# endernewton/tf-faster-rcnn

Measured on AMD Instinct MI355X. Metric: images/sec (600×1000) ResNet-101 Faster R-CNN at 1/2/4/8 MI355X, higher is better.
Workload: dtype f32 (operands, accumulators, results; GEMMs with Cin, Cout % 128 == 0 form each f32 product from two-piece fp16 operands with an exact power-of-two scale per 128-k block on the fp16 matrix pipe -- 3 MFMAs / product, dropped terms <= 3 * 2^-22, measured error vs float64 below the f32-MFMA kernel's; o

## Files before the change

### include/frcnn_hip.h

```cpp
#ifndef FRCNN_HIP_H_
#define FRCNN_HIP_H_
#include <stddef.h>
#include <stdint.h>

#ifdef __cplusplus
extern "C" {
#endif

#define FRCNN_OK 0
#define FRCNN_E_ARG (-1)
#define FRCNN_E_WS (-2)
#define FRCNN_E_UNSUPPORTED (-3)
#define FRCNN_E_HIP(e) (-(1000 + (int)(e)))

#define FRCNN_NMS_RULE_CPU 0
#define FRCNN_NMS_RULE_GPU 1

#define FRCNN_ACT_NONE 0
#define FRCNN_ACT_RELU 1
#define FRCNN_ACT_RELU6 2

#define FRCNN_ABI_VERSION 6
int frcnn_abi_version(void);
const char* frcnn_build_info(void);
// ... 63 lines not shown
int frcnn_detect_post_batched(const float* cls_prob_d, const float* bbox_pred_d, const float* rois_d, const int* num_rois_d,
                              int B, int R, int C, double im_scale, int im_h, int im_w, double nms_thresh, int rule,
                              float score_thresh, int max_per_image, float* out_dets_d, int* out_count_d, int max_out,
                              long long out_stride, void* ws, size_t ws_bytes, void* stream);

int frcnn_im_detect_boxes(const float* rois_d, const float* bbox_pred_d, int R, int C, double im_scale,
                          int im_h, int im_w, float* boxes_d, void* stream);

int frcnn_bbox_transform_inv(const float* boxes_d, const float* deltas_d, int N, int k, float* out_d, void* stream);
int frcnn_clip_boxes(float* boxes_d, int N, int k, float im_h, float im_w, void* stream);
int frcnn_bbox_transform(const float* ex_rois_d, const float* gt_rois_d, int N, float* targets_d, void* stream);

int frcnn_bbox_overlaps(const double* boxes_d, int n, const double* query_d, int k, double* out_d, void* stream);

size_t frcnn_coco_match_workspace_bytes(int n_groups, long long n_det, long long n_gt, long long n_pairs);
int frcnn_coco_match(const double* det_xywh_d, const long long* det_off_d, const double* gt_xywh_d, const double* gt_area_d,
                     const unsigned char* gt_crowd_d, const long long* gt_off_d, int n_groups, const double* iou_thrs_d, int T,
                     const double* area_rng_d, int A, unsigned char* det_matched_d, unsigned char* det_ignored_d,
                     unsigned char* gt_ignored_d, double* iou_out_d, void* ws, size_t ws_bytes, void* stream);

int frcnn_conv2d_nhwc(const float* x_d, int N, int H, int W, int Cin, const float* w_d, const float* bias_d,
                      const float* residual_d, int RH, int RW, int res_stride, float* y_d, int OH, int OW,
                      int Cout, int KH, int KW, int stride, int pad_top, int pad_left, int act, int fold_w,
                      void* stream);
size_t frcnn_conv2d_workspace_bytes(int N, int OH, int OW, int Cout, int KH, int KW, int Cin, int fold_w);
int frcnn_conv2d_nhwc_ws(const float* x_d, int N, int H, int W, int Cin, const float* w_d, const float* bias_d,
                         const float* residual_d, int RH, int RW, int res_stride, float* y_d, int OH, int OW, int Cout, int KH,
                         int KW, int stride, int pad_top, int pad_left, int act, int fold_w, void* ws, size_t ws_bytes,
                         void* stream);

int frcnn_set_tuning(int key, int value);
unsigned int frcnn_crc32c(const void* data, size_t n, unsigned int crc);

long long frcnn_snappy_uncompress(const unsigned char* src, size_t n, unsigned char* dst, size_t cap);

int frcnn_prep_image_shape(int h, int w, int target_size, int max_size, double* im_scale, int* out_h, int* out_w);
int frcnn_prep_image(const void* src_d, int src_is_float, int h, int w, const double* pixel_means, double im_scale, float* out_d,
                     int OH, int OW, int out_c, void* stream);
int frcnn_prep_image_batched(const void* src_d, int src_is_float, int B, int h, int w, const double* pixel_means, double im_scale,
                             float* out_d, int OH, int OW, int out_c, void* stream);
int frcnn_prep_train_image(const void* src_d, int src_is_float, int h, int w, int flipped, const double* pixel_means, double im_scale,
                           float* out_d, int OH, int OW, int out_c, const unsigned short* boxes_d, const int* classes_d, int G,
                           float* gt_d, void* stream);

int frcnn_jpeg_info(const unsigned char* data, size_t n, int* out8);
size_t frcnn_jpeg_coef_bytes(int width, int height, int ncomp, int hs, int vs);
int frcnn_jpeg_entropy_decode(const unsigned char* data, size_t n, void* coef_h, size_t coef_bytes);
int frcnn_jpeg_pixels_host(const void* coef_h, int width, int height, int ncomp, int hs, int vs, unsigned char* bgr_h);
size_t frcnn_jpeg_workspace_bytes(int width, int height, int ncomp, int hs, int vs);
int frcnn_jpeg_pixels(const void* coef_d, int width, int height, int ncomp, int hs, int vs, unsigned char* bgr_d, void* ws,
                      size_t ws_bytes, void* stream);

int frcnn_gemm_batched_nt(const float* x_d, const float* w_d, float* y_d, int G, int M, int N, int K, void* stream);
size_t frcnn_gemm_x3_pack_bytes(int G, int N, int K);
int frcnn_gemm_x3_pack(const float* w_d, int G, int N, int K, void* planes_d, void* stream);
int frcnn_gemm_x3(const float* x_d, const void* planes_d, const float* bias_d, const float* res_d, float* y_d, int G, int M, int N,
                  int K, int act, int cfg, int terms, void* stream);
size_t frcnn_h2_planes_bytes(long long rows, int K);
int frcnn_h2_pack_w(const float* w_d, int G, int N, int K, void* planes_d, float* w_inv_d, void* stream);
int frcnn_h2_split(const float* x_d, long long M, int K, void* planes_d, float* inv_d, void* stream);
int frcnn_gemm_h2(const void* x_planes_d, const float* x_inv_d, const void* w_planes_d, const float* w_inv_d, const float* bias_d,
                  const float* res_d, const void* res_planes_d, const float* res_inv_d, float* y_d, void* y_planes_d, float* y_inv_d,
                  int G, int M, int N, int K, int act, int cfg, void* stream);
size_t frcnn_gemm_h2_mean_workspace_bytes(int G, int M, int N);
int frcnn_gemm_h2_mean(const void* x_planes_d, const float* x_inv_d, const void* w_planes_d, const float* w_inv_d, const float* bias_d,
                       const float* res_d, const void* res_planes_d, const float* res_inv_d, int G, int M, int N, int K, int act, int rows,
                       float* mean_out_d, void* ws, size_t ws_bytes, int cfg, void* stream);
int frcnn_winograd_filter_transform(const float* w_hwio, int Cin, int Cout, const float* scale, int m, float* u_out);
int frcnn_winograd_filter_transform_device(const float* w_packed_d, int Cout, int Cin, int m, int transpose_flip, float* u_d,
                                           void* stream);
int frcnn_winograd_input_transform(const float* x_d, int N, int H, int W, int C, int m, float* v_d, void* stream);
int frcnn_winograd_output_transform(const float* m_d, int N, int H, int W, int C, int m, const float* bias_d, int act, float* y_d,
                                    void* stream);
int frcnn_winograd7_filter_transform(const float* w_hwio, int Cin, int Cout, const float* scale, float* u_out);
int frcnn_winograd7_filter_transform_device(const float* w_packed_d, int Cout, int Cin, int transpose_flip, float* u_d, void* stream);
int frcnn_winograd7_input_transform(const float* x_d, int R, int C, float* v_d, void* stream);
int frcnn_winograd7_output_transform(const float* m_d, int R, int C, const float* bias_d, int act, float* y_d, void* stream);
int frcnn_winograd_input_transform_h2(const float* x_d, int N, int H, int W, int C, int m, void* v_planes_d, float* v_inv_d, void* stream);
int frcnn_winograd_output_transform_h2(const float* m_d, int N, int H, int W, int C, int m, const float* bias_d, int act, float* y_d,
                                       void* y_planes_d, float* y_inv_d, void* stream);
int frcnn_winograd7_input_transform_h2(const float* x_d, int R, int C, void* v_planes_d, float* v_inv_d, void* stream);
int frcnn_winograd7_output_transform_h2(const float* m_d, int R, int C, const float* bias_d, int act, float* y_d, void* y_planes_d,
                                        float* y_inv_d, void* stream);
int frcnn_pack_filter_hwio(const float* w_hwio, int KH, int KW, int Cin, int Cout, const float* scale, float* out);
int frcnn_maxpool_nhwc(const float* x_d, int N, int H, int W, int C, int k, int stride, int pad_top,
                       int pad_left, float* y_d, int OH, int OW, void* stream);
int frcnn_dwconv3x3_nhwc(const float* x_d, int N, int H, int W, int C, const float* w_d, const float* bias_d,
                         float* y_d, int OH, int OW, int stride, int pad_top, int pad_left, int act, void* stream);
int frcnn_dwconv3x3_nhwc_h2(const float* x_d, int N, int H, int W, int C, const float* w_d, const float* bias_d, float* y_d,
                            void* y_planes_d, float* y_inv_d, int OH, int OW, int stride, int pad_top, int pad_left, int act, void* stream);
int frcnn_spatial_mean(const float* x_d, int N, int HW, int C, float* y_d, void* stream);
int frcnn_softmax_rows(const float* x_d, int R, int C, int ld, float* y_d, void* stream);
int frcnn_rpn_softmax(const float* score_d, int HW, int A, int ld, float* prob_d, void* stream);
int frcnn_copy_cols(const float* src_d, int R, int ld_src, int col0, int cols, float* dst_d, int ld_dst, void* stream);

size_t frcnn_anchor_target_workspace_bytes(int H, int W, int A, int max_gt);
int frcnn_anchor_target_layer(const float* gt_boxes_d, int G, float im_h, float im_w, int H, int W, int A,
                              int feat_stride, const double* base_d, int rpn_batchsize, double fg_fraction,
                              double pos_overlap, double neg_overlap, long long seed, const double* opts, float* labels_d,
                              float* bbox_targets_d, float* inside_w_d, float* outside_w_d, void* ws,
                              size_t ws_bytes, void* stream);
int frcnn_anchor_target_layer_inject(const float* gt_boxes_d, int G, float im_h, float im_w, int H, int W, int A, int feat_stride,
                                     const double* base_d, int rpn_batchsize, double fg_fraction, double pos_overlap,
                                     double neg_overlap, const int* disable_d, int n_disable, const double* opts, float* labels_d,
                                     float* bbox_targets_d, float* inside_w_d, float* outside_w_d, void* ws, size_t ws_bytes,
                                     void* stream);
int frcnn_proposal_target_layer(const float* rpn_rois_d, const float* rpn_scores_d, int N, const float* gt_boxes_d,
                                int G, int num_classes, int batch_size, double fg_fraction, double fg_thresh,
                                double bg_thresh_hi, double bg_thresh_lo, const double* means4, const double* stds4,
                                long long seed, const double* opts, float* rois_d, float* roi_scores_d, float* labels_d,
                                float* bbox_targets_d, float* inside_w_d, float* outside_w_d, int* counts_d,
                                void* stream);
int frcnn_proposal_target_layer_dn(const float* rpn_rois_d, const float* rpn_scores_d, int max_rois, const int* num_rois_d,
                                   const float* gt_boxes_d, int G, int num_classes, int batch_size, double fg_fraction,
                                   double fg_thresh, double bg_thresh_hi, double bg_thresh_lo, const double* means4,
                                   const double* stds4, long long seed, const double* opts, float* rois_d, float* roi_scores_d,
                                   float* labels_d, float* bbox_targets_d, float* inside_w_d, float* outside_w_d, int* counts_d,
                                   void* stream);
int frcnn_proposal_target_layer_inject(const float* rpn_rois_d, const float* rpn_scores_d, int N, const float* gt_boxes_d, int G,
                                       int num_classes, int batch_size, const int* keep_inds_d, int n_fg, const double* means4,
                                       const double* stds4, const double* opts, float* rois_d, float* roi_scores_d, float* labels_d,
                                       float* bbox_targets_d, float* inside_w_d, float* outside_w_d, void* stream);
size_t frcnn_loss_workspace_bytes(long long elements);
int frcnn_softmax_ce_loss(const float* logits_d, const float* labels_d, int R, int C, int rpn_A, int rpn_H, int rpn_W,
                          float* loss_d, float* dlogits_d, void* ws, size_t ws_bytes, void* stream);
int frcnn_smooth_l1_loss(const float* pred_d, const float* targets_d, const float* inside_w_d, const float* outside_w_d,
                         long long n, float sigma, float mean_divisor, float* loss_d, float* dpred_d, void* ws,
                         size_t ws_bytes, void* stream);

int frcnn_transpose_pad(const float* in_d, int M, int C, float* out_d, int Mp, void* stream);
int frcnn_im2col_t(const float* x_d, int N, int H, int W, int Cin, int OH, int OW, int KH, int KW, int stride,
                   int pad_top, int pad_left, float* out_d, int Mp, void* stream);
int frcnn_flip_transpose_filter(const float* w_d, int Cout, int KH, int KW, int Cin, float* out_d, void* stream);
int frcnn_conv2d_dgrad_strided(const float* dy_d, int N, int OH, int OW, int Cout, const float* w_d, int KH, int KW,
                               int Cin, int stride, int pad_top, int pad_left, float* dx_d, int H, int W,
                               int accumulate, void* stream);
int frcnn_conv2d_wgrad_supported(int Cin, int Cout);
size_t frcnn_conv2d_wgrad_workspace_bytes(int N, int OH, int OW, int Cin, int Cout, int KH, int KW);
int frcnn_conv2d_wgrad(const float* dy_d, const float* x_d, int N, int H, int W, int Cin, int OH, int OW, int Cout, int KH, int KW,
                       int stride, int pad_top, int pad_left, float* dw_d, void* ws, size_t ws_bytes, void* stream);
void frcnn_conv2d_wgrad_set_plan(int tile, int min_workgroups);
size_t frcnn_conv2d_wgrad_h2_workspace_bytes(int N, int OH, int OW, int Cin, int Cout, int KH, int KW);
int frcnn_conv2d_wgrad_h2(const float* dy_d, const float* x_d, int N, int H, int W, int Cin, int OH, int OW, int Cout, int KH, int KW,
                          int stride, int pad_top, int pad_left, float* dw_d, void* ws, size_t ws_bytes, void* stream);
void frcnn_conv2d_wgrad_h2_set_plan(int tile, int min_workgroups);
int frcnn_relu_bwd(float* grad_d, const float* y_d, long long n, void* stream);
int frcnn_conv2d_nhwc_masked_ws(const float* x_d, int N, int H, int W, int Cin, const float* w_d, const float* bias_d,
                                const float* residual_d, int RH, int RW, int res_stride, float* y_d, int OH, int OW,
                                int Cout, int KH, int KW, int stride, int pad_top, int pad_left, int act, const float* mask_d,
                                void* ws, size_t ws_bytes, void* stream);
int frcnn_gemm_h2_masked(const void* x_planes_d, const float* x_inv_d, const void* w_planes_d, const float* w_inv_d, const float* bias_d,
                         const float* res_d, const float* mask_d, float* y_d, void* y_planes_d, float* y_inv_d, int G, int M, int N, int K,
                         int act, int cfg, void* stream);
int frcnn_winograd_output_transform_masked(const float* m_d, int N, int H, int W, int C, int m, const float* mask_d, float* y_d,
                                           void* y_planes_d, float* y_inv_d, void* stream);
int frcnn_winograd7_output_transform_masked(const float* m_d, int R, int C, const float* mask_d, float* y_d, void* y_planes_d,
                                            float* y_inv_d, void* stream);
int frcnn_relu6_bwd(float* grad_d, const float* y_d, long long n, void* stream);
int frcnn_maxpool_bwd(const float* x_d, int N, int H, int W, int C, int k, int stride, const float* y_d, const float* dy_d,
                      int OH, int OW, float* dx_d, void* stream);
int frcnn_dropout(const float* x_d, long long n, unsigned long long seed, float keep_prob, float* y_d, void* stream);
int frcnn_dwconv3x3_dgrad(const float* g_d, int N, int OH, int OW, int C, const float* w_d, float* dx_d, int H, int W, int stride,
                          int pad_top, int pad_left, int accumulate, void* stream);
size_t frcnn_dwconv3x3_wgrad_workspace_bytes(int N, int OH, int OW, int C);
int frcnn_dwconv3x3_wgrad(const float* g_d, const float* x_d, int N, int H, int W, int C, int OH, int OW, int stride, int pad_top,
                          int pad_left, const float* scale_d, float* dw_d, void* ws, size_t ws_bytes, void* stream);
// ... 41 lines not shown
```

### tf-faster-rcnn_amd/csrc/detect_kernels.hip

```cpp
#include "common.h"

extern "C" int frcnn_generate_anchors(int base_size, const double* ratios, int n_ratios, const double* scales,
                                      int n_scales, double* out_base) {
  if (!ratios || !scales || !out_base || n_ratios <= 0 || n_scales <= 0 || base_size <= 0) return FRCNN_E_ARG;
  const double w = (double)base_size, h = (double)base_size;
  const double cx = 0.5 * (w - 1), cy = 0.5 * (h - 1);
  for (int r = 0; r < n_ratios; ++r) {
    const double ws = nearbyint(sqrt(w * h / ratios[r]));
    const double hs = nearbyint(ws * ratios[r]);
    const double x1 = cx - 0.5 * (ws - 1), y1 = cy - 0.5 * (hs - 1);
    const double x2 = cx + 0.5 * (ws - 1), y2 = cy + 0.5 * (hs - 1);
    const double aw = x2 - x1 + 1, ah = y2 - y1 + 1;
    const double acx = x1 + 0.5 * (aw - 1), acy = y1 + 0.5 * (ah - 1);
    for (int s = 0; s < n_scales; ++s) {
      const double sw = aw * scales[s], sh = ah * scales[s];
      double* o = out_base + 4 * ((size_t)r * n_scales + s);
      o[0] = acx - 0.5 * (sw - 1);
      o[1] = acy - 0.5 * (sh - 1);
      o[2] = acx + 0.5 * (sw - 1);
      o[3] = acy + 0.5 * (sh - 1);
    }
  }
  return FRCNN_OK;
}

__device__ __forceinline__ float4 anchor_at(const double* __restrict__ base, int n, int A, int W, int stride) {
  const int a = n % A, pix = n / A;
  const double sx = (double)((pix % W) * stride), sy = (double)((pix / W) * stride);
  const double* b = base + 4 * a;
  return make_float4((float)(b[0] + sx), (float)(b[1] + sy), (float)(b[2] + sx), (float)(b[3] + sy));
}

__global__ void k_anchors(const double* __restrict__ base, int A, int W, int stride, int N, float4* __restrict__ out) {
  const int n = blockIdx.x * blockDim.x + threadIdx.x;
  if (n < N) out[n] = anchor_at(base, n, A, W, stride);
}

extern "C" int frcnn_generate_anchors_pre(int height, int width, int feat_stride, const double* base_d, int A,
                                          float* anchors_d, void* stream) {
  if (!base_d || !anchors_d || height <= 0 || width <= 0 || A <= 0) return FRCNN_E_ARG;
  const int N = height * width * A;
  hipLaunchKernelGGL(k_anchors, dim3(cdiv(N, 256)), dim3(256), 0, (hipStream_t)stream, base_d, A, width,
                     feat_stride, N, (float4*)anchors_d);
  LAUNCH_CHECK();
  return FRCNN_OK;
}

#define NMS_RULE_CPU FRCNN_NMS_RULE_CPU
#define NMS_RULE_GPU FRCNN_NMS_RULE_GPU
#define NMS_RULE_TF 2

__global__ void k_decode_clip_key(const float* __restrict__ prob, const float4* __restrict__ deltas,
                                  const double* __restrict__ base, int A, int W, int stride, int N, float hi_x,
                                  float hi_y, float4* __restrict__ boxes, u64* __restrict__ keys, size_t img) {
  const int n = blockIdx.x * blockDim.x + threadIdx.x;
  if (n >= N) return;
  const int b = blockIdx.y;
  prob += (size_t)b * 2 * N;
  deltas += (size_t)b * N;
  const int a = n % A, pix = n / A;
  const float score = prob[(size_t)pix * 2 * A + A + a];
  float4 bx = decode_box(anchor_at(base, n, A, W, stride), deltas[n]);
  bx.x = rmax(rmin(bx.x, hi_x), 0.0f);
  bx.y = rmax(rmin(bx.y, hi_y), 0.0f);
  bx.z = rmax(rmin(bx.z, hi_x), 0.0f);
  bx.w = rmax(rmin(bx.w, hi_y), 0.0f);
  img_ptr(boxes, img, b)[n] = bx;
  img_ptr(keys, img, b)[n] = make_key(score, (u32)n);
}

__global__ void k_dets_key(const float* __restrict__ dets, int k, float4* __restrict__ boxes, u64* __restrict__ keys) {
  const int n = blockIdx.x * blockDim.x + threadIdx.x;
  if (n >= k) return;
  const float* d = dets + 5 * (size_t)n;
  boxes[n] = make_float4(d[0], d[1], d[2], d[3]);
  keys[n] = make_key(d[4], (u32)n);
}

__global__ void k_boxes_scores_key(const float4* __restrict__ in_boxes, const float* __restrict__ in_scores, int k,
                                   float4* __restrict__ boxes, u64* __restrict__ keys) {
  const int n = blockIdx.x * blockDim.x + threadIdx.x;
  if (n >= k) return;
  boxes[n] = in_boxes[n];
// ... 652 lines not shown
  if (!rpn_cls_prob_d || !rpn_bbox_pred_d || !base_d || !rois_d || !scores_d || !ws) return FRCNN_E_ARG;
  if (H <= 0 || W <= 0 || A <= 0 || rpn_top_n <= 0) return FRCNN_E_ARG;
  const int N = H * W * A;
  if (N < rpn_top_n) return FRCNN_E_UNSUPPORTED;
  hipStream_t st = (hipStream_t)stream;
  SortWs s = carve(ws, N, rpn_top_n);
  if (s.bytes > ws_bytes) return FRCNN_E_WS;
  int rc = launch_decode(s, rpn_cls_prob_d, rpn_bbox_pred_d, 1, im_h, im_w, W, A, feat_stride, base_d, N, st);
  if (rc) return rc;
  rc = launch_topk_sort(s, N, rpn_top_n, 1, st);
  if (rc) return rc;
  hipLaunchKernelGGL(k_top_rois, dim3(cdiv(rpn_top_n, 256)), dim3(256), 0, st, s.sboxes, s.sscores, rpn_top_n, rois_d,
                     scores_d);
  LAUNCH_CHECK();
  return FRCNN_OK;
}

extern "C" int frcnn_proposal_top_layer_inds(const float* rpn_cls_prob_d, const float* rpn_bbox_pred_d, float im_h, float im_w,
                                             int H, int W, int A, int feat_stride, const double* base_d, const int* top_inds_d,
                                             int n_inds, float* rois_d, float* scores_d, void* stream) {
  if (!rpn_cls_prob_d || !rpn_bbox_pred_d || !base_d || !rois_d || !scores_d || !top_inds_d) return FRCNN_E_ARG;
  if (H <= 0 || W <= 0 || A <= 0 || n_inds <= 0) return FRCNN_E_ARG;
  hipLaunchKernelGGL(k_decode_gather, dim3(cdiv(n_inds, 256)), dim3(256), 0, (hipStream_t)stream, rpn_cls_prob_d,
                     (const float4*)rpn_bbox_pred_d, base_d, A, W, feat_stride, H * W * A, im_w - 1.0f, im_h - 1.0f, top_inds_d, n_inds,
                     rois_d, scores_d);
  LAUNCH_CHECK();
  return FRCNN_OK;
}

extern "C" int frcnn_non_max_suppression(const float* boxes_d, const float* scores_d, int k, int max_output_size,
                                         float iou_threshold, int* selected_d, int* num_d, void* ws, size_t ws_bytes,
                                         void* stream) {
  if (!num_d || k < 0 || max_output_size < 0) return FRCNN_E_ARG;
  hipStream_t st = (hipStream_t)stream;
  if (k == 0 || max_output_size == 0) {
    HIP_TRY(hipMemsetAsync(num_d, 0, sizeof(int), st));
    return FRCNN_OK;
  }
  if (!boxes_d || !scores_d || !selected_d || !ws) return FRCNN_E_ARG;
  if (k > NMS_MAX_BOXES) return FRCNN_E_UNSUPPORTED;
  SortWs s = carve(ws, k, k);
  if (s.bytes > ws_bytes) return FRCNN_E_WS;
  hipLaunchKernelGGL(k_boxes_scores_key, dim3(cdiv(k, 256)), dim3(256), 0, st, (const float4*)boxes_d, scores_d, k, s.boxes,
                     s.keys);
  LAUNCH_CHECK();
  int rc = launch_topk_sort(s, k, k, 1, st);
  if (rc) return rc;
  rc = launch_mask(s, k, 1, iou_threshold, NMS_RULE_TF, st);
  if (rc) return rc;
  ReduceOut o = {s.sboxes, s.sscores, s.sidx, nullptr, nullptr, selected_d, num_d, 0};
  return launch_reduce(s, k, 1, min(max_output_size, k), o, st);
}

extern "C" int frcnn_proposal_layer_tf_batched(const float* rpn_cls_prob_d, const float* rpn_bbox_pred_d, int B, float im_h,
                                               float im_w, int H, int W, int A, int feat_stride, const double* base_d,
                                               int post_nms_topn, float nms_thresh, float* rois_d, float* scores_d, int* num_d,
                                               void* ws, size_t ws_bytes, void* stream) {
  if (!rpn_cls_prob_d || !rpn_bbox_pred_d || !base_d || !rois_d || !scores_d || !num_d || !ws) return FRCNN_E_ARG;
  if (B <= 0 || H <= 0 || W <= 0 || A <= 0 || post_nms_topn <= 0) return FRCNN_E_ARG;
  const long long NN = (long long)H * W * A;
  if (NN > NMS_MAX_BOXES) return FRCNN_E_UNSUPPORTED;
  const int N = (int)NN;
  hipStream_t st = (hipStream_t)stream;
  SortWs s = carve(ws, N, N);
  if (s.bytes * (size_t)B > ws_bytes) return FRCNN_E_WS;
  int rc = launch_decode(s, rpn_cls_prob_d, rpn_bbox_pred_d, B, im_h, im_w, W, A, feat_stride, base_d, N, st);
  if (rc) return rc;
  rc = launch_topk_sort(s, N, N, B, st);
  if (rc) return rc;
  rc = launch_mask(s, N, B, nms_thresh, NMS_RULE_TF, st);
  if (rc) return rc;
  ReduceOut o = {s.sboxes, s.sscores, s.sidx, rois_d, scores_d, nullptr, num_d, 1};
  return launch_reduce(s, N, B, post_nms_topn, o, st);
}

extern "C" int frcnn_proposal_layer_tf(const float* rpn_cls_prob_d, const float* rpn_bbox_pred_d, float im_h, float im_w,
                                       int H, int W, int A, int feat_stride, const double* base_d, int post_nms_topn,
                                       float nms_thresh, float* rois_d, float* scores_d, int* num_d, void* ws,
                                       size_t ws_bytes, void* stream) {
  return frcnn_proposal_layer_tf_batched(rpn_cls_prob_d, rpn_bbox_pred_d, 1, im_h, im_w, H, W, A, feat_stride, base_d, post_nms_topn,
                                         nms_thresh, rois_d, scores_d, num_d, ws, ws_bytes, stream);
}

__device__ __forceinline__ float4 lerp4(const float4 a, const float4 b, float t) {
  return make_float4(a.x + (b.x - a.x) * t, a.y + (b.y - a.y) * t, a.z + (b.z - a.z) * t, a.w + (b.w - a.w) * t);
}
__device__ __forceinline__ float4 max4(const float4 a, const float4 b) {
  return make_float4(fmaxf(a.x, b.x), fmaxf(a.y, b.y), fmaxf(a.z, b.z), fmaxf(a.w, b.w));
}

__device__ __forceinline__ float4 crop_sample(const float4* __restrict__ feat, int H, int W, int C4, int c4, float y1,
                                              float x1, float hs, float ws, int gy, int gx) {
  const float in_y = y1 * (float)(H - 1) + (float)gy * hs;
  const float in_x = x1 * (float)(W - 1) + (float)gx * ws;
  if (in_y < 0 || in_y > (float)(H - 1) || in_x < 0 || in_x > (float)(W - 1)) return make_float4(0, 0, 0, 0);
  const int top = (int)floorf(in_y), bot = (int)ceilf(in_y);
  const int left = (int)floorf(in_x), right = (int)ceilf(in_x);
  const float ly = in_y - (float)top, lx = in_x - (float)left;
  const float4 tl = feat[((size_t)top * W + left) * C4 + c4], tr = feat[((size_t)top * W + right) * C4 + c4];
  const float4 bl = feat[((size_t)bot * W + left) * C4 + c4], br = feat[((size_t)bot * W + right) * C4 + c4];
  return lerp4(lerp4(tl, tr, lx), lerp4(bl, br, lx), ly);
}

template <bool MAX2>
__global__ __launch_bounds__(256) void k_crop_and_resize(const float4* __restrict__ feat_all, int NIMG, int H, int W, int C4,
                                                         int nslab, const float* __restrict__ rois, float stride, int pool,
                                                         const float4* __restrict__ bias, int act, float4* __restrict__ out) {
  const int slab = blockIdx.x % nslab, rp = blockIdx.x / nslab;
  const int r = rp / pool, py = rp % pool;
  const int SC4 = C4 / nslab, c40 = slab * SC4;
  const float height = ((float)H - 1.0f) * stride, width = ((float)W - 1.0f) * stride;
  const float* roi = rois + 5 * (size_t)r;
  const int img = (int)roi[0];
  float4* orow = out + ((size_t)r * pool + py) * pool * C4;
  if (img < 0 || img >= NIMG) {
    for (int t = threadIdx.x; t < pool * SC4; t += 256) orow[(size_t)(t / SC4) * C4 + c40 + t % SC4] = make_float4(0, 0, 0, 0);
    return;
  }
  const float4* feat = feat_all + (size_t)img * H * W * C4;
  const float x1 = roi[1] / width, y1 = roi[2] / height, x2 = roi[3] / width, y2 = roi[4] / height;
  const int P = MAX2 ? 2 * pool : pool;
  const float hs = (y2 - y1) * (float)(H - 1) / (float)(P - 1);
  const float ws = (x2 - x1) * (float)(W - 1) / (float)(P - 1);
  for (int t = threadIdx.x; t < pool * SC4; t += 256) {
    const int px = t / SC4, c4 = c40 + t % SC4;
    float4 v;
    if (MAX2) {
      v = crop_sample(feat, H, W, C4, c4, y1, x1, hs, ws, 2 * py, 2 * px);
      v = max4(v, crop_sample(feat, H, W, C4, c4, y1, x1, hs, ws, 2 * py, 2 * px + 1));
      v = max4(v, crop_sample(feat, H, W, C4, c4, y1, x1, hs, ws, 2 * py + 1, 2 * px));
      v = max4(v, crop_sample(feat, H, W, C4, c4, y1, x1, hs, ws, 2 * py + 1, 2 * px + 1));
    } else {
      v = crop_sample(feat, H, W, C4, c4, y1, x1, hs, ws, py, px);
    }
    if (bias) {
      const float4 bv = bias[c4];
      v.x += bv.x; v.y += bv.y; v.z += bv.z; v.w += bv.w;
    }
    if (act == FRCNN_ACT_RELU) v = act_relu(v);
    orow[(size_t)px * C4 + c4] = v;
  }
}

template <bool MAX2, int ITEMS>
__global__ __launch_bounds__(256) void k_crop_and_resize_roi(const float4* __restrict__ feat_all, int NIMG, int H, int W, int C4,
                                                             int nslab, const float* __restrict__ rois, float stride, int pool,
                                                             const float4* __restrict__ bias, int act, float4* __restrict__ out) {
  const int slab = blockIdx.x % nslab, r = blockIdx.x / nslab;
  const int SC4 = C4 / nslab, c40 = slab * SC4;
  const float height = ((float)H - 1.0f) * stride, width = ((float)W - 1.0f) * stride;
  const float* roi = rois + 5 * (size_t)r;
  const int img = (int)roi[0];
  float4* obase = out + (size_t)r * pool * pool * C4;
  const int total = pool * pool * SC4;
  if (img < 0 || img >= NIMG) {
    for (int t = threadIdx.x; t < total; t += 256) obase[(size_t)(t / SC4) * C4 + c40 + t % SC4] = make_float4(0, 0, 0, 0);
    return;
  }
  const float4* feat = feat_all + (size_t)img * H * W * C4;
  const float x1 = roi[1] / width, y1 = roi[2] / height, x2 = roi[3] / width, y2 = roi[4] / height;
  const int P = MAX2 ? 2 * pool : pool;
  const float hs = (y2 - y1) * (float)(H - 1) / (float)(P - 1);
  const float ws = (x2 - x1) * (float)(W - 1) / (float)(P - 1);
  for (int t0 = threadIdx.x; t0 < total; t0 += 256 * ITEMS) {
    float4 v[ITEMS];
#pragma unroll
    for (int k = 0; k < ITEMS; ++k) {
      const int t = t0 + k * 256;
      if (t >= total) { v[k] = make_float4(0, 0, 0, 0); continue; }
      const int pix = t / SC4, c4 = c40 + t % SC4;
      const int py = pix / pool, px = pix - py * pool;
      if (MAX2) {
        v[k] = crop_sample(feat, H, W, C4, c4, y1, x1, hs, ws, 2 * py, 2 * px);
        v[k] = max4(v[k], crop_sample(feat, H, W, C4, c4, y1, x1, hs, ws, 2 * py, 2 * px + 1));
        v[k] = max4(v[k], crop_sample(feat, H, W, C4, c4, y1, x1, hs, ws, 2 * py + 1, 2 * px));
        v[k] = max4(v[k], crop_sample(feat, H, W, C4, c4, y1, x1, hs, ws, 2 * py + 1, 2 * px + 1));
      } else {
        v[k] = crop_sample(feat, H, W, C4, c4, y1, x1, hs, ws, py, px);
      }
    }
#pragma unroll
    for (int k = 0; k < ITEMS; ++k) {
      const int t = t0 + k * 256;
      if (t >= total) continue;
      const int pix = t / SC4, c4 = c40 + t % SC4;
      float4 o = v[k];
      if (bias) {
        const float4 bv = bias[c4];
        o.x += bv.x; o.y += bv.y; o.z += bv.z; o.w += bv.w;
      }
      if (act == FRCNN_ACT_RELU) o = act_relu(o);
      obase[(size_t)pix * C4 + c4] = o;
    }
  }
}

static thread_local int g_crop_slabs = -1;
static thread_local int g_crop_form = 0;

static int launch_crop(const float* feat_d, int NIMG, int H, int W, int C, const float* rois_d, int R, float feat_stride, int pool,
                       int fuse_max2x2, const float* bias_d, int act, float* out_d, void* stream) {
  if (R == 0) return FRCNN_OK;
  if (!feat_d || !rois_d || !out_d || NIMG <= 0 || H < 2 || W < 2 || C <= 0 || R < 0 || pool < 2) return FRCNN_E_ARG;
  if (C % 4) return FRCNN_E_UNSUPPORTED;
  hipStream_t st = (hipStream_t)stream;
  const int C4 = C / 4;
  int nslab = (C4 % 8 == 0 && C4 / 8 >= 16) ? 8 : 1;
  if (g_crop_form == 0 && nslab == 8 && C4 / 8 < 32) nslab = 4;
  if (g_crop_slabs > 0 && C4 % g_crop_slabs == 0) nslab = g_crop_slabs;
  const long long blocks = (long long)R * pool * nslab;
  if (blocks >= (1ll << 31)) return FRCNN_E_UNSUPPORTED;
  if (g_crop_form == 0) {
    const unsigned grid = (unsigned)((long long)R * nslab);
    if (fuse_max2x2)
      hipLaunchKernelGGL((k_crop_and_resize_roi<true, 2>), dim3(grid), dim3(256), 0, st, (const float4*)feat_d, NIMG, H, W, C4, nslab, rois_d,
                         feat_stride, pool, (const float4*)bias_d, act, (float4*)out_d);
    else
      hipLaunchKernelGGL((k_crop_and_resize_roi<false, 4>), dim3(grid), dim3(256), 0, st, (const float4*)feat_d, NIMG, H, W, C4, nslab, rois_d,
                         feat_stride, pool, (const float4*)bias_d, act, (float4*)out_d);
    LAUNCH_CHECK();
    return FRCNN_OK;
  }
  if (fuse_max2x2)
    hipLaunchKernelGGL(k_crop_and_resize<true>, dim3((unsigned)blocks), dim3(256), 0, st, (const float4*)feat_d, NIMG, H, W, C4, nslab,
                       rois_d, feat_stride, pool, (const float4*)bias_d, act, (float4*)out_d);
  else
    hipLaunchKernelGGL(k_crop_and_resize<false>, dim3((unsigned)blocks), dim3(256), 0, st, (const float4*)feat_d, NIMG, H, W, C4, nslab,
                       rois_d, feat_stride, pool, (const float4*)bias_d, act, (float4*)out_d);
  LAUNCH_CHECK();
  return FRCNN_OK;
}

extern "C" int frcnn_detect_set_tuning(int key, int value) {
  if (key == 4) { g_crop_slabs = value; return FRCNN_OK; }
  if (key == 5) { g_crop_form = value; return FRCNN_OK; }
  return FRCNN_E_ARG;
}

extern "C" int frcnn_crop_and_resize(const float* feat_d, int H, int W, int C, const float* rois_d, int R,
                                     float feat_stride, int pool, int fuse_max2x2, float* out_d, void* stream) {
  return launch_crop(feat_d, 1, H, W, C, rois_d, R, feat_stride, pool, fuse_max2x2, nullptr, FRCNN_ACT_NONE, out_d, stream);
}

extern "C" int frcnn_crop_and_resize_batched(const float* feat_d, int N, int H, int W, int C, const float* rois_d, int R,
                                             float feat_stride, int pool, int fuse_max2x2, float* out_d, void* stream) {
  return launch_crop(feat_d, N, H, W, C, rois_d, R, feat_stride, pool, fuse_max2x2, nullptr, FRCNN_ACT_NONE, out_d, stream);
}

extern "C" int frcnn_crop_and_resize_bias_act(const float* feat_d, int N, int H, int W, int C, const float* rois_d, int R,
                                              float feat_stride, int pool, const float* bias_d, int act, float* out_d,
                                              void* stream) {
  if (act != FRCNN_ACT_NONE && act != FRCNN_ACT_RELU) return FRCNN_E_ARG;
  return launch_crop(feat_d, N, H, W, C, rois_d, R, feat_stride, pool, 0, bias_d, act, out_d, stream);
}

__global__ void k_bbox_transform_inv(const float4* __restrict__ boxes, const float4* __restrict__ deltas, int N, int k,
                                     float4* __restrict__ out) {
  const long long t = (long long)blockIdx.x * blockDim.x + threadIdx.x;
  if (t >= (long long)N * k) return;
  out[t] = decode_box(boxes[t / k], deltas[t]);
}
__global__ void k_clip_boxes(float4* __restrict__ boxes, long long n, float hi_x, float hi_y) {
  const long long t = (long long)blockIdx.x * blockDim.x + threadIdx.x;
  if (t >= n) return;
  float4 b = boxes[t];
  b.x = rmax(rmin(b.x, hi_x), 0.0f); b.y = rmax(rmin(b.y, hi_y), 0.0f);
  b.z = rmax(rmin(b.z, hi_x), 0.0f); b.w = rmax(rmin(b.w, hi_y), 0.0f);
  boxes[t] = b;
}
__global__ void k_bbox_transform(const float4* __restrict__ ex, const float4* __restrict__ gt, int N, float4* __restrict__ out) {
  const int t = blockIdx.x * blockDim.x + threadIdx.x;
  if (t >= N) return;
  const float4 e = ex[t], g = gt[t];
  const float ew = (e.z - e.x) + 1.0f, eh = (e.w - e.y) + 1.0f;
  const float ecx = e.x + 0.5f * ew, ecy = e.y + 0.5f * eh;
  const float gw = (g.z - g.x) + 1.0f, gh = (g.w - g.y) + 1.0f;
  const float gcx = g.x + 0.5f * gw, gcy = g.y + 0.5f * gh;
  out[t] = make_float4((gcx - ecx) / ew, (gcy - ecy) / eh, logf(gw / ew), logf(gh / eh));
}

extern "C" int frcnn_bbox_transform_inv(const float* boxes_d, const float* deltas_d, int N, int k, float* out_d, void* stream) {
  if (N < 0 || k <= 0) return FRCNN_E_ARG;
  if (N == 0) return FRCNN_OK;
  if (!boxes_d || !deltas_d || !out_d) return FRCNN_E_ARG;
  const long long tot = (long long)N * k;
  hipLaunchKernelGGL(k_bbox_transform_inv, dim3((unsigned)((tot + 255) / 256)), dim3(256), 0, (hipStream_t)stream,
                     (const float4*)boxes_d, (const float4*)deltas_d, N, k, (float4*)out_d);
  LAUNCH_CHECK();
  return FRCNN_OK;
}
extern "C" int frcnn_clip_boxes(float* boxes_d, int N, int k, float im_h, float im_w, void* stream) {
// ... 299 lines not shown
```

### tf-faster-rcnn_amd/csrc/gemm_h2.hip

```cpp
#include "h2_common.h"
#include <mutex>
#include <type_traits>

typedef float f32x16 __attribute__((ext_vector_type(16)));
typedef _Float16 h8 __attribute__((ext_vector_type(8)));

#define LDS_AS __attribute__((address_space(3)))

struct GemmH2Params {
  const unsigned short* x; const float* x_inv; const unsigned short* w; const float* w_inv;
  const float* bias; const float* res; const unsigned short* resp; const float* resp_inv; float* y; unsigned short* yp; float* y_inv;
  int M, N, K, batch, act, nsteps, mtiles, ntiles;
  long long Mtot;
  int wshare;
  const float* mask;
  float* mean_part; int mean_rows;
};

__device__ __forceinline__ void h2_glds16(unsigned voff, const void* sbase, unsigned lds_base) {
  unsigned keep;
  asm volatile(
      "s_mov_b32 %0, m0\n\t"
      "s_mov_b32 m0, %3\n\t"
      "s_nop 0\n\t"
// ... 1028 lines not shown
  return FRCNN_OK;
}

template <int MASK>
static int h2_dispatch(const GemmH2Params& p, int cfg, hipStream_t st) {
  switch (cfg) {
    case 9: return launch_h2<128, 128, 64, 64, 2, 2, H2_SCALES_ONCE + MASK>(p, st);
    case 12: return launch_h2<64, 128, 32, 64, 2, 2, MASK>(p, st);
    case 21: return launch_h2<256, 128, 64, 64, 3, 2, H2_SCALES_ONCE + H2_PINGPONG + MASK>(p, st);
    case 30: return launch_h2<128, 128, 64, 64, 2, 2, H2_SCALES_ONCE + H2_LIGHT_BOUNDARY + MASK>(p, st);
    case 31: return launch_h2<128, 128, 64, 64, 2, 2, H2_SCALES_ONCE + H2_LIGHT_BOUNDARY + H2_STORE16 + MASK>(p, st);
    case 32: return launch_h2<128, 128, 64, 64, 2, 2, H2_SCALES_ONCE + H2_STORE16 + MASK>(p, st);
    case 33: return launch_h2<64, 128, 32, 64, 2, 2, H2_LIGHT_BOUNDARY + H2_STORE16 + MASK>(p, st);
    case 34: return launch_h2<256, 128, 64, 64, 3, 2, H2_SCALES_ONCE + H2_PINGPONG + H2_STORE16 + MASK>(p, st);
    case 40: return launch_h2<128, 128, 64, 64, 2, 2, H2_SCALES_ONCE + H2_LIGHT_BOUNDARY + H2_STORE16 + H2_DEFERRED + MASK>(p, st);
    case 41: return launch_h2<64, 128, 32, 64, 2, 2, H2_LIGHT_BOUNDARY + H2_STORE16 + H2_DEFERRED + MASK>(p, st);
  }
#ifdef FRCNN_ABLATION
  constexpr int CFG31 = H2_SCALES_ONCE + H2_LIGHT_BOUNDARY + H2_STORE16;
  if constexpr (MASK == 0) switch (cfg) {
    case 50: return launch_h2<128, 128, 64, 64, 2, 2, CFG31 + H2_NO_MFMA>(p, st);
    case 51: return launch_h2<128, 128, 64, 64, 2, 2, CFG31 + H2_NO_FRAG>(p, st);
    case 52: return launch_h2<128, 128, 64, 64, 2, 2, CFG31 + H2_NO_LOAD>(p, st);
    case 53: return launch_h2<128, 128, 64, 64, 2, 2, CFG31 + H2_NO_MFMA + H2_NO_FRAG>(p, st);
    case 54: return launch_h2<128, 128, 64, 64, 2, 2, CFG31 + H2_NO_FRAG + H2_NO_LOAD>(p, st);
    case 55: return launch_h2<128, 128, 64, 64, 2, 2, CFG31 + H2_NO_MFMA + H2_NO_FRAG + H2_NO_LOAD>(p, st);
  }
#endif
  return FRCNN_E_ARG;
}

static int run_h2(GemmH2Params& p, int cfg, hipStream_t st);

static GemmH2Params h2_params(const void* x_planes_d, const float* x_inv_d, const void* w_planes_d, const float* w_inv_d, const float* bias_d,
                              const float* res_d, const void* res_planes_d, const float* res_inv_d, float* y_d, void* y_planes_d, float* y_inv_d,
                              int G, int M, int N, int K, int act) {
  GemmH2Params p;
  p.x = (const unsigned short*)x_planes_d; p.x_inv = x_inv_d; p.w = (const unsigned short*)w_planes_d; p.w_inv = w_inv_d;
  p.bias = bias_d; p.res = res_d; p.resp = (const unsigned short*)res_planes_d; p.resp_inv = res_inv_d; p.y = y_d; p.yp = (unsigned short*)y_planes_d; p.y_inv = y_inv_d;
  p.M = M; p.N = N; p.K = K; p.batch = G; p.act = act; p.Mtot = (long long)G * M;
  p.nsteps = p.mtiles = p.ntiles = 0;
  p.mean_part = nullptr; p.mean_rows = 0; p.wshare = 0; p.mask = nullptr;
  return p;
}

extern "C" int frcnn_gemm_h2(const void* x_planes_d, const float* x_inv_d, const void* w_planes_d, const float* w_inv_d, const float* bias_d,
                             const float* res_d, const void* res_planes_d, const float* res_inv_d, float* y_d, void* y_planes_d, float* y_inv_d,
                             int G, int M, int N, int K, int act, int cfg, void* stream) {
  if (!x_planes_d || !x_inv_d || !w_planes_d || !w_inv_d || (!y_d && !y_planes_d) || (y_planes_d && !y_inv_d) || G <= 0 || M <= 0 || N <= 0 ||
      K <= 0 || act < 0 || act > 2 || (res_d && res_planes_d) || (res_planes_d && !res_inv_d))
    return FRCNN_E_ARG;
  const long long Mtot = (long long)G * M;
  if (K % H2_KB || N % 128 || 4ll * Mtot * K >= (1ll << 32) || 4ll * N * K >= (1ll << 32) ||
      (long long)M * N >= (1ll << 29))
    return FRCNN_E_UNSUPPORTED;
  GemmH2Params p = h2_params(x_planes_d, x_inv_d, w_planes_d, w_inv_d, bias_d, res_d, res_planes_d, res_inv_d, y_d, y_planes_d, y_inv_d, G, M, N, K, act);
  return run_h2(p, cfg, (hipStream_t)stream);
}

extern "C" int frcnn_gemm_h2_masked(const void* x_planes_d, const float* x_inv_d, const void* w_planes_d, const float* w_inv_d, const float* bias_d,
                                    const float* res_d, const float* mask_d, float* y_d, void* y_planes_d, float* y_inv_d, int G, int M, int N, int K,
                                    int act, int cfg, void* stream) {
  if (!x_planes_d || !x_inv_d || !w_planes_d || !w_inv_d || !mask_d || (!y_d && !y_planes_d) || (y_planes_d && !y_inv_d) || G <= 0 || M <= 0 ||
      N <= 0 || K <= 0 || act < 0 || act > 2)
    return FRCNN_E_ARG;
  const long long Mtot = (long long)G * M;
  if (K % H2_KB || N % 128 || 4ll * Mtot * K >= (1ll << 32) || 4ll * N * K >= (1ll << 32) || (long long)M * N >= (1ll << 29)) return FRCNN_E_UNSUPPORTED;
  GemmH2Params p = h2_params(x_planes_d, x_inv_d, w_planes_d, w_inv_d, bias_d, res_d, nullptr, nullptr, y_d, y_planes_d, y_inv_d, G, M, N, K, act);
  p.mask = mask_d;
  return run_h2(p, cfg, (hipStream_t)stream);
}

static int run_h2(GemmH2Params& p, int cfg, hipStream_t st) {
  const int G = p.batch, M = p.M, N = p.N, K = p.K;
  if (cfg < 0) {
    const long long mt256 = (M + 255) / 256;
#ifndef FRCNN_H2_PP_MIN_K
#define FRCNN_H2_PP_MIN_K 1024
#endif
    const int pp_min_k = ((cfg == -4 || cfg == -5 || cfg == -6) && !p.mean_part) ? 512 : FRCNN_H2_PP_MIN_K;
    const int pp_cfg = (cfg == -3 || cfg == -4 || (cfg == -6 && K < FRCNN_H2_PP_MIN_K)) ? 34 : 21;
    const bool pp = K >= pp_min_k && mt256 * 256 * 100 <= (long long)M * 104 && mt256 * (N / 128) * G >= 256;
    const bool tiny = (long long)((M + 127) / 128) * (N / 128) * G < 150;
    const bool de = cfg != -2 && cfg != -7 && !p.mean_part && !p.mask && ((p.resp && p.yp && !p.y) || cfg == -8);
    cfg = pp ? pp_cfg : tiny ? (cfg == -2 ? 12 : (de && cfg == -8) ? 41 : 33) : (cfg == -2 ? 9 : de ? 40 : 31);
  }
  if (p.mean_part && (cfg == 40 || cfg == 41)) cfg = cfg == 40 ? 31 : 33;
  return p.mask ? h2_dispatch<H2_MASKED>(p, cfg, st) : h2_dispatch<0>(p, cfg, st);
}

__global__ __launch_bounds__(256) void k_h2_mean_finish(const float* __restrict__ part, int G, int M, int N4, int rows, float4* __restrict__ out) {
  const long long t = (long long)blockIdx.x * blockDim.x + threadIdx.x;
  const int per = M / rows;
  if (t >= (long long)G * per * N4) return;
  const int n4 = (int)(t % N4);
  const long long gr = t / N4;
  const int g = (int)(gr / per), r = (int)(gr % per);
  const int nblk = (M + 31) >> 5;
  const int row0 = r * rows, row1 = row0 + rows - 1;
  float4 s = make_float4(0.f, 0.f, 0.f, 0.f);
  for (int b = row0 >> 5; b <= (row1 >> 5); ++b) {
    const int which = ((b << 5) / rows == r) ? 0 : 1;
    const float4 v = *(const float4*)(part + (((size_t)g * nblk + b) * 2 + which) * (size_t)N4 * 4 + (size_t)n4 * 4);
    s.x += v.x; s.y += v.y; s.z += v.z; s.w += v.w;
  }
  const float inv = 1.0f / (float)rows;
  out[t] = make_float4(s.x * inv, s.y * inv, s.z * inv, s.w * inv);
}

extern "C" size_t frcnn_gemm_h2_mean_workspace_bytes(int G, int M, int N) {
  if (G <= 0 || M <= 0 || N <= 0) return 256;
  return (size_t)G * (size_t)((M + 31) / 32) * 2 * (size_t)N * sizeof(float);
}

extern "C" int frcnn_gemm_h2_mean(const void* x_planes_d, const float* x_inv_d, const void* w_planes_d, const float* w_inv_d, const float* bias_d,
                                  const float* res_d, const void* res_planes_d, const float* res_inv_d, int G, int M, int N, int K, int act, int rows,
                                  float* mean_out_d, void* ws, size_t ws_bytes, int cfg, void* stream) {
  if (!x_planes_d || !x_inv_d || !w_planes_d || !w_inv_d || !mean_out_d || !ws || G <= 0 || M <= 0 || N <= 0 || K <= 0 || act < 0 || act > 2 ||
      rows <= 0 || (res_d && res_planes_d) || (res_planes_d && !res_inv_d))
    return FRCNN_E_ARG;
  const long long Mtot = (long long)G * M;
  if (K % H2_KB || N % 128 || M % rows || rows < 32 || 4ll * Mtot * K >= (1ll << 32) || 4ll * N * K >= (1ll << 32) || (long long)M * N >= (1ll << 29))
    return FRCNN_E_UNSUPPORTED;
  if (frcnn_gemm_h2_mean_workspace_bytes(G, M, N) > ws_bytes) return FRCNN_E_WS;
  GemmH2Params p = h2_params(x_planes_d, x_inv_d, w_planes_d, w_inv_d, bias_d, res_d, res_planes_d, res_inv_d, nullptr, nullptr, nullptr, G, M, N, K, act);
  p.mean_part = (float*)ws; p.mean_rows = rows; p.wshare = 1;
  hipStream_t st = (hipStream_t)stream;
  const int rc = run_h2(p, cfg, st);
  if (rc) return rc;
  const long long tot = (long long)G * (M / rows) * (N / 4);
  hipLaunchKernelGGL(k_h2_mean_finish, dim3((unsigned)((tot + 255) / 256)), dim3(256), 0, st, (const float*)ws, G, M, N / 4, rows, (float4*)mean_out_d);
  LAUNCH_CHECK();
  return FRCNN_OK;
}
```

### tf-faster-rcnn_amd/csrc/winograd7.hip

```cpp
#include "h2_common.h"

namespace w7 {
constexpr float BT[11][9] = {
    {4.f, 0.f, -5.f, 0.f, 1.f, 0.f, 0.f, 0.f, 0.f},  {0.f, -4.f, -4.f, 1.f, 1.f, 0.f, 0.f, 0.f, 0.f}, {0.f, 4.f, -4.f, -1.f, 1.f, 0.f, 0.f, 0.f, 0.f},
    {0.f, -2.f, -1.f, 2.f, 1.f, 0.f, 0.f, 0.f, 0.f}, {0.f, 2.f, -1.f, -2.f, 1.f, 0.f, 0.f, 0.f, 0.f}, {0.f, 4.f, 0.f, -5.f, 0.f, 1.f, 0.f, 0.f, 0.f},
    {0.f, 0.f, 0.f, 0.f, 2.f, -1.f, -2.f, 1.f, 0.f}, {0.f, 0.f, 0.f, 0.f, 0.f, -2.f, -1.f, 1.f, 0.f}, {0.f, 0.f, 0.f, 0.f, 0.f, 2.f, -3.f, 1.f, 0.f},
    {0.f, 0.f, 0.f, 0.f, 0.f, -1.f, 0.f, 1.f, 0.f},  {0.f, 0.f, 0.f, 0.f, 0.f, 2.f, -1.f, -2.f, 1.f}};
constexpr float AT[7][11] = {
    {1.f, 1.f, 1.f, 1.f, 1.f, 0.f, 0.f, 0.f, 0.f, 0.f, 0.f},  {0.f, 1.f, -1.f, 2.f, -2.f, 0.f, 0.f, 0.f, 0.f, 0.f, 0.f},
    {0.f, 1.f, 1.f, 4.f, 4.f, 0.f, 0.f, 0.f, 0.f, 0.f, 0.f},  {0.f, 1.f, -1.f, 8.f, -8.f, 1.f, 0.f, 0.f, 0.f, 0.f, 0.f},
    {0.f, 0.f, 0.f, 0.f, 0.f, 0.f, 1.f, 1.f, 1.f, 1.f, 0.f},  {0.f, 0.f, 0.f, 0.f, 0.f, 0.f, 0.f, 1.f, -1.f, 2.f, 0.f},
    {0.f, 0.f, 0.f, 0.f, 0.f, 0.f, 0.f, 1.f, 1.f, 4.f, 1.f}};
constexpr double G[11][3] = {{1.0 / 4, 0, 0},          {-1.0 / 6, -1.0 / 6, -1.0 / 6}, {-1.0 / 6, 1.0 / 6, -1.0 / 6}, {1.0 / 24, 1.0 / 12, 1.0 / 6},
                             {1.0 / 24, -1.0 / 12, 1.0 / 6}, {0, 0, 1},                {1.0 / 2, 0, 0},               {-1.0 / 2, -1.0 / 2, -1.0 / 2},
                             {-1.0 / 6, 1.0 / 6, -1.0 / 6},  {1.0 / 6, 1.0 / 3, 2.0 / 3}, {0, 0, 1}};
}

__device__ __forceinline__ float2 f2mad(float a, float2 x, float2 y) { return make_float2(a * x.x + y.x, a * x.y + y.y); }

__device__ __forceinline__ void acc_term(float2& acc, bool& first, float coef, const float2 x) {
  if (coef == 0.f) return;
  if (first) {
    acc = coef == 1.f ? x : (coef == -1.f ? make_float2(-x.x, -x.y) : make_float2(coef * x.x, coef * x.y));
    first = false;
  } else if (coef == 1.f) {
    acc = make_float2(acc.x + x.x, acc.y + x.y);
  } else if (coef == -1.f) {
    acc = make_float2(acc.x - x.x, acc.y - x.y);
  } else {
    acc = f2mad(coef, x, acc);
  }
}

template <bool H2>
struct Wino7Sink {
  float2* f; unsigned short* planes; float* inv; size_t rows;
  template <int NR>
  __device__ __forceinline__ void putn(const size_t* row, const float2* v, int c2, int C2) const {
    if (!H2 || f) {
#pragma unroll
      for (int n = 0; n < NR; ++n) f[row[n] * C2 + c2] = v[n];
    }
    if (H2) {
      size_t e[NR];
      float* slot[NR];
#pragma unroll
      for (int n = 0; n < NR; ++n) {
        e[n] = (row[n] * C2 + c2) * 2;
        slot[n] = inv + (size_t)(c2 >> 6) * rows + row[n];
      }
      h2_emit_rows64<NR>(v, e, slot, (1u << NR) - 1u, planes, rows * (size_t)C2 * 2, c2 & 63);
    }
  }
};

template <bool H2>
__global__ void __launch_bounds__(256) k_wino7_input(const float2* __restrict__ x, int R, int C2, const Wino7Sink<H2> V) {
  const long long id = (long long)blockIdx.x * blockDim.x + threadIdx.x;
  if (id >= (long long)R * C2) return;
  const int c2 = (int)(id % C2);
  const int r = (int)(id / C2);
  float2 d[7][7];
  const float2* src = x + (size_t)r * 49 * C2 + c2;
#pragma unroll
  for (int i = 0; i < 7; ++i)
#pragma unroll
    for (int j = 0; j < 7; ++j) d[i][j] = src[(size_t)(i * 7 + j) * C2];
#pragma unroll
  for (int xi = 0; xi < 11; ++xi) {
    float2 t[7];
#pragma unroll
    for (int j = 0; j < 7; ++j) {
      bool first = true;
      t[j] = make_float2(0.f, 0.f);
#pragma unroll
      for (int i = 0; i < 7; ++i) acc_term(t[j], first, w7::BT[xi][i + 1], d[i][j]);
    }
    float2 o[11];
    size_t rw[11];
#pragma unroll
    for (int nu = 0; nu < 11; ++nu) {
      bool first = true;
      float2 v = make_float2(0.f, 0.f);
#pragma unroll
      for (int j = 0; j < 7; ++j) acc_term(v, first, w7::BT[nu][j + 1], t[j]);
      o[nu] = v;
      rw[nu] = (size_t)(xi * 11 + nu) * R + r;
    }
    V.template putn<11>(rw, o, c2, C2);
  }
}

template <int XI0, int NXI, int I0, int NI, bool H2, bool MASK>
__device__ __forceinline__ void wino7_out_segment(const float2* __restrict__ in, size_t plane, float2 bv, int act, const Wino7Sink<H2>& y,
                                                  size_t row0, int c2, int C2, const float2* __restrict__ mask) {
  float2 m[NXI][11];
#pragma unroll
  for (int a = 0; a < NXI; ++a)
#pragma unroll
    for (int nu = 0; nu < 11; ++nu) m[a][nu] = in[(size_t)((XI0 + a) * 11 + nu) * plane];
#pragma unroll
  for (int i = 0; i < NI; ++i) {
    float2 s[11];
#pragma unroll
    for (int nu = 0; nu < 11; ++nu) {
      bool first = true;
      s[nu] = make_float2(0.f, 0.f);
#pragma unroll
      for (int a = 0; a < NXI; ++a) acc_term(s[nu], first, w7::AT[I0 + i][XI0 + a], m[a][nu]);
    }
    float2 o[7];
    size_t rw[7];
#pragma unroll
    for (int j = 0; j < 7; ++j) {
      bool first = true;
      float2 v = make_float2(0.f, 0.f);
#pragma unroll
      for (int nu = 0; nu < 11; ++nu) acc_term(v, first, w7::AT[j][nu], s[nu]);
      v = make_float2(v.x + bv.x, v.y + bv.y);
      if (act == FRCNN_ACT_RELU) v = act_relu(v);
      rw[j] = row0 + (I0 + i) * 7 + j;
      if (MASK) {
        const float2 k = mask[rw[j] * C2 + c2];
        v.x = k.x > 0.f ? v.x : 0.f; v.y = k.y > 0.f ? v.y : 0.f;
      }
      o[j] = v;
    }
    y.template putn<7>(rw, o, c2, C2);
  }
}

template <bool H2, bool MASK = false>
__global__ void __launch_bounds__(256) k_wino7_output(const float2* __restrict__ Mx, int R, int C2, const float2* __restrict__ bias, int act,
                                                       const float2* __restrict__ mask, const Wino7Sink<H2> y) {
  const long long id = (long long)blockIdx.x * blockDim.x + threadIdx.x;
  if (id >= (long long)R * C2) return;
  const int c2 = (int)(id % C2);
  const int r = (int)(id / C2);
  const size_t plane = (size_t)R * C2;
  const float2* in = Mx + (size_t)r * C2 + c2;
  const float2 bv = bias ? bias[c2] : make_float2(0.f, 0.f);
  wino7_out_segment<0, 6, 0, 4, H2, MASK>(in, plane, bv, act, y, (size_t)r * 49, c2, C2, mask);
  wino7_out_segment<6, 5, 4, 3, H2, MASK>(in, plane, bv, act, y, (size_t)r * 49, c2, C2, mask);
}

__global__ void k_wino7_filter(const float* __restrict__ w, int O, int C, int transpose_flip, float* __restrict__ U) {
  const long long id = (long long)blockIdx.x * blockDim.x + threadIdx.x;
  if (id >= (long long)O * C) return;
  int o, c;
  if (transpose_flip) { o = (int)(id % O); c = (int)(id / O); }
  else { c = (int)(id % C); o = (int)(id / C); }
  float g[3][3];
#pragma unroll
  for (int i = 0; i < 3; ++i)
#pragma unroll
    for (int j = 0; j < 3; ++j) {
      const int kh = transpose_flip ? 2 - i : i, kw = transpose_flip ? 2 - j : j;
      g[i][j] = w[(((size_t)o * 3 + kh) * 3 + kw) * C + c];
    }
  float t[11][3];
#pragma unroll
  for (int a = 0; a < 11; ++a)
#pragma unroll
    for (int j = 0; j < 3; ++j) t[a][j] = (float)w7::G[a][0] * g[0][j] + (float)w7::G[a][1] * g[1][j] + (float)w7::G[a][2] * g[2][j];
  const size_t plane = (size_t)O * C;
  float* out = U + (transpose_flip ? (size_t)c * O + o : (size_t)o * C + c);
#pragma unroll
  for (int a = 0; a < 11; ++a)
#pragma unroll
    for (int b = 0; b < 11; ++b)
      out[(size_t)(a * 11 + b) * plane] = t[a][0] * (float)w7::G[b][0] + t[a][1] * (float)w7::G[b][1] + t[a][2] * (float)w7::G[b][2];
}

extern "C" int frcnn_winograd7_filter_transform(const float* w_hwio, int Cin, int Cout, const float* scale, float* u_out) {
  if (!w_hwio || !u_out || Cin <= 0 || Cout <= 0) return FRCNN_E_ARG;
  for (int c = 0; c < Cin; ++c)
    for (int o = 0; o < Cout; ++o) {
      double g[3][3], t[11][3];
      const double sc = scale ? (double)scale[o] : 1.0;
      for (int i = 0; i < 3; ++i)
        for (int j = 0; j < 3; ++j) g[i][j] = (double)w_hwio[((size_t)(i * 3 + j) * Cin + c) * Cout + o] * sc;
      for (int a = 0; a < 11; ++a)
        for (int j = 0; j < 3; ++j) t[a][j] = w7::G[a][0] * g[0][j] + w7::G[a][1] * g[1][j] + w7::G[a][2] * g[2][j];
      for (int a = 0; a < 11; ++a)
        for (int b = 0; b < 11; ++b)
          u_out[((size_t)(a * 11 + b) * Cout + o) * Cin + c] = (float)(t[a][0] * w7::G[b][0] + t[a][1] * w7::G[b][1] + t[a][2] * w7::G[b][2]);
    }
  return FRCNN_OK;
}

extern "C" int frcnn_winograd7_filter_transform_device(const float* w_packed_d, int Cout, int Cin, int transpose_flip, float* u_d,
                                                       void* stream) {
  if (!w_packed_d || !u_d || Cout <= 0 || Cin <= 0) return FRCNN_E_ARG;
  const long long tot = (long long)Cout * Cin;
  hipLaunchKernelGGL(k_wino7_filter, dim3((unsigned)((tot + 255) / 256)), dim3(256), 0, (hipStream_t)stream, w_packed_d, Cout, Cin,
                     transpose_flip ? 1 : 0, u_d);
  LAUNCH_CHECK();
  return FRCNN_OK;
}

extern "C" int frcnn_winograd7_input_transform(const float* x_d, int R, int C, float* v_d, void* stream) {
  if (!x_d || !v_d || R <= 0 || C <= 0) return FRCNN_E_ARG;
  if (C % 2) return FRCNN_E_UNSUPPORTED;
  const long long tot = (long long)R * (C / 2);
  const Wino7Sink<false> sink{(float2*)v_d, nullptr, nullptr, 0};
  hipLaunchKernelGGL(k_wino7_input<false>, dim3((unsigned)((tot + 255) / 256)), dim3(256), 0, (hipStream_t)stream, (const float2*)x_d, R, C / 2, sink);
  LAUNCH_CHECK();
  return FRCNN_OK;
}

extern "C" int frcnn_winograd7_input_transform_h2(const float* x_d, int R, int C, void* v_planes_d, float* v_inv_d, void* stream) {
  if (!x_d || !v_planes_d || !v_inv_d || R <= 0 || C <= 0) return FRCNN_E_ARG;
  if (C % H2_KB) return FRCNN_E_UNSUPPORTED;
  const long long tot = (long long)R * (C / 2);
  const Wino7Sink<true> sink{nullptr, (unsigned short*)v_planes_d, v_inv_d, (size_t)121 * R};
  hipLaunchKernelGGL(k_wino7_input<true>, dim3((unsigned)((tot + 255) / 256)), dim3(256), 0, (hipStream_t)stream, (const float2*)x_d, R, C / 2, sink);
  LAUNCH_CHECK();
  return FRCNN_OK;
}

extern "C" int frcnn_winograd7_output_transform(const float* m_d, int R, int C, const float* bias_d, int act, float* y_d, void* stream) {
  if (!m_d || !y_d || R <= 0 || C <= 0) return FRCNN_E_ARG;
  if (C % 2 || (act != FRCNN_ACT_NONE && act != FRCNN_ACT_RELU)) return FRCNN_E_UNSUPPORTED;
  const long long tot = (long long)R * (C / 2);
  const Wino7Sink<false> sink{(float2*)y_d, nullptr, nullptr, 0};
  hipLaunchKernelGGL((k_wino7_output<false, false>), dim3((unsigned)((tot + 255) / 256)), dim3(256), 0, (hipStream_t)stream, (const float2*)m_d, R,
                     C / 2, (const float2*)bias_d, act, (const float2*)nullptr, sink);
  LAUNCH_CHECK();
  return FRCNN_OK;
}

extern "C" int frcnn_winograd7_output_transform_h2(const float* m_d, int R, int C, const float* bias_d, int act, float* y_d, void* y_planes_d,
                                                   float* y_inv_d, void* stream) {
  if (!m_d || !y_planes_d || !y_inv_d || R <= 0 || C <= 0) return FRCNN_E_ARG;
  if (C % H2_KB || (act != FRCNN_ACT_NONE && act != FRCNN_ACT_RELU)) return FRCNN_E_UNSUPPORTED;
  const long long tot = (long long)R * (C / 2);
  const Wino7Sink<true> sink{(float2*)y_d, (unsigned short*)y_planes_d, y_inv_d, (size_t)R * 49};
  hipLaunchKernelGGL((k_wino7_output<true, false>), dim3((unsigned)((tot + 255) / 256)), dim3(256), 0, (hipStream_t)stream, (const float2*)m_d, R,
                     C / 2, (const float2*)bias_d, act, (const float2*)nullptr, sink);
  LAUNCH_CHECK();
  return FRCNN_OK;
}

extern "C" int frcnn_winograd7_output_transform_masked(const float* m_d, int R, int C, const float* mask_d, float* y_d, void* y_planes_d,
                                                       float* y_inv_d, void* stream) {
  if (!m_d || !mask_d || (!y_d && !y_planes_d) || (y_planes_d && !y_inv_d) || R <= 0 || C <= 0) return FRCNN_E_ARG;
  if (C % 2 || (y_planes_d && C % H2_KB)) return FRCNN_E_UNSUPPORTED;
  const long long tot = (long long)R * (C / 2);
  if (y_planes_d) {
    const Wino7Sink<true> sink{(float2*)y_d, (unsigned short*)y_planes_d, y_inv_d, (size_t)R * 49};
    hipLaunchKernelGGL((k_wino7_output<true, true>), dim3((unsigned)((tot + 255) / 256)), dim3(256), 0, (hipStream_t)stream, (const float2*)m_d, R,
                       C / 2, (const float2*)nullptr, FRCNN_ACT_NONE, (const float2*)mask_d, sink);
  } else {
    const Wino7Sink<false> sink{(float2*)y_d, nullptr, nullptr, 0};
    hipLaunchKernelGGL((k_wino7_output<false, true>), dim3((unsigned)((tot + 255) / 256)), dim3(256), 0, (hipStream_t)stream, (const float2*)m_d, R,
                       C / 2, (const float2*)nullptr, FRCNN_ACT_NONE, (const float2*)mask_d, sink);
  }
  LAUNCH_CHECK();
  return FRCNN_OK;
}
```

### tf-faster-rcnn_amd/frcnn_hip/__init__.py

```python
import ctypes
import os
from ctypes import c_double, c_float, c_int, c_longlong, c_size_t, c_ulonglong, c_void_p

_PKG = os.path.dirname(os.path.abspath(__file__))
LIB_PATH = os.path.join(_PKG, "libfrcnn_hip.so")
_lib = None

ABI_VERSION = 6
ACT_NONE, ACT_RELU, ACT_RELU6 = 0, 1, 2
NMS_RULE_CPU, NMS_RULE_GPU = 0, 1

_P = c_void_p
SIGNATURES = {
    "frcnn_abi_version": (c_int, []),
    "frcnn_build_info": (ctypes.c_char_p, []),
    "_nms": (None, [_P, _P, _P, c_int, c_int, c_float, c_int]),
    "frcnn_nms_workspace_bytes": (c_size_t, [c_int]),
    "frcnn_nms": (c_int, [_P, c_int, c_double, c_int, _P, _P, _P, c_size_t, _P]),
    "frcnn_nms_sorted": (c_int, [_P, c_int, c_int, c_double, c_int, _P, _P, _P, c_size_t, _P]),
    "frcnn_nms_rule": (c_int, [_P, c_int, c_double, c_int, c_int, _P, _P, _P, c_size_t, _P]),
    "frcnn_nms_sorted_rule": (c_int, [_P, c_int, c_int, c_double, c_int, c_int, _P, _P, _P, c_size_t, _P]),
    "frcnn_generate_anchors": (c_int, [c_int, _P, c_int, _P, c_int, _P]),
    "frcnn_generate_anchors_pre": (c_int, [c_int, c_int, c_int, _P, c_int, _P, _P]),
    "frcnn_proposal_workspace_bytes": (c_size_t, [c_int, c_int, c_int, c_int]),
    "frcnn_proposal_layer": (c_int, [_P, _P, c_float, c_float, c_int, c_int, c_int, c_int, _P, c_int, c_int, c_double,
                                     _P, _P, _P, _P, c_size_t, _P]),
    "frcnn_proposal_batched_workspace_bytes": (c_size_t, [c_int, c_int, c_int, c_int, c_int]),
    "frcnn_proposal_layer_batched": (c_int, [_P, _P, c_int, c_float, c_float, c_int, c_int, c_int, c_int, _P, c_int, c_int, c_double,
                                             c_int, _P, _P, _P, _P, c_size_t, _P]),
    "frcnn_proposal_top_layer_inds": (c_int, [_P, _P, c_float, c_float, c_int, c_int, c_int, c_int, _P, _P, c_int, _P, _P, _P]),
    "frcnn_proposal_layer_tf_batched": (c_int, [_P, _P, c_int, c_float, c_float, c_int, c_int, c_int, c_int, _P, c_int, c_float, _P, _P,
                                                _P, _P, c_size_t, _P]),
    "frcnn_proposal_top_layer": (c_int, [_P, _P, c_float, c_float, c_int, c_int, c_int, c_int, _P, c_int, _P, _P, _P,
                                         c_size_t, _P]),
    "frcnn_non_max_suppression": (c_int, [_P, _P, c_int, c_int, c_float, _P, _P, _P, c_size_t, _P]),
    "frcnn_proposal_layer_tf": (c_int, [_P, _P, c_float, c_float, c_int, c_int, c_int, c_int, _P, c_int, c_float, _P, _P, _P,
                                        _P, c_size_t, _P]),
    "frcnn_crop_and_resize": (c_int, [_P, c_int, c_int, c_int, _P, c_int, c_float, c_int, c_int, _P, _P]),
    "frcnn_crop_and_resize_batched": (c_int, [_P, c_int, c_int, c_int, c_int, _P, c_int, c_float, c_int, c_int, _P, _P]),
    "frcnn_crop_and_resize_bias_act": (c_int, [_P, c_int, c_int, c_int, c_int, _P, c_int, c_float, c_int, _P, c_int, _P, _P]),
    "frcnn_detect_set_tuning": (c_int, [c_int, c_int]),
    "frcnn_detect_post_batched_workspace_bytes": (c_size_t, [c_int, c_int, c_int]),
    "frcnn_detect_post_batched": (c_int, [_P, _P, _P, _P, c_int, c_int, c_int, c_double, c_int, c_int, c_double, c_int, c_float, c_int,
                                          _P, _P, c_int, c_longlong, _P, c_size_t, _P]),
    "frcnn_detect_post_workspace_bytes": (c_size_t, [c_int, c_int]),
    "frcnn_detect_post": (c_int, [_P, _P, _P, _P, c_int, c_int, c_double, c_int, c_int, c_double, c_float, c_int, _P, _P,
                                  c_int, _P, c_size_t, _P]),
    "frcnn_im_detect_boxes": (c_int, [_P, _P, c_int, c_int, c_double, c_int, c_int, _P, _P]),
    "frcnn_bbox_overlaps": (c_int, [_P, c_int, _P, c_int, _P, _P]),
    "frcnn_coco_match_workspace_bytes": (c_size_t, [c_int, c_longlong, c_longlong, c_longlong]),
    "frcnn_coco_match": (c_int, [_P, _P, _P, _P, _P, _P, c_int, _P, c_int, _P, c_int, _P, _P, _P, _P, _P, c_size_t, _P]),
    "frcnn_bbox_transform_inv": (c_int, [_P, _P, c_int, c_int, _P, _P]),
    "frcnn_clip_boxes": (c_int, [_P, c_int, c_int, c_float, c_float, _P]),
    "frcnn_bbox_transform": (c_int, [_P, _P, c_int, _P, _P]),
    "frcnn_conv2d_nhwc": (c_int, [_P, c_int, c_int, c_int, c_int, _P, _P, _P, c_int, c_int, c_int, _P, c_int, c_int,
                                  c_int, c_int, c_int, c_int, c_int, c_int, c_int, c_int, _P]),
    "frcnn_conv2d_workspace_bytes": (c_size_t, [c_int, c_int, c_int, c_int, c_int, c_int, c_int, c_int]),
    "frcnn_conv2d_nhwc_ws": (c_int, [_P, c_int, c_int, c_int, c_int, _P, _P, _P, c_int, c_int, c_int, _P, c_int, c_int,
                                     c_int, c_int, c_int, c_int, c_int, c_int, c_int, c_int, _P, c_size_t, _P]),
    "frcnn_conv2d_nhwc_masked_ws": (c_int, [_P, c_int, c_int, c_int, c_int, _P, _P, _P, c_int, c_int, c_int, _P, c_int, c_int,
                                            c_int, c_int, c_int, c_int, c_int, c_int, c_int, _P, _P, c_size_t, _P]),
    "frcnn_gemm_h2_masked": (c_int, [_P, _P, _P, _P, _P, _P, _P, _P, _P, _P, c_int, c_int, c_int, c_int, c_int, c_int, _P]),
    "frcnn_winograd_output_transform_masked": (c_int, [_P, c_int, c_int, c_int, c_int, c_int, _P, _P, _P, _P, _P]),
    "frcnn_winograd7_output_transform_masked": (c_int, [_P, c_int, c_int, _P, _P, _P, _P, _P]),
    "frcnn_crc32c": (ctypes.c_uint32, [_P, c_size_t, ctypes.c_uint32]),
    "frcnn_snappy_uncompress": (c_longlong, [_P, c_size_t, _P, c_size_t]),
    "frcnn_prep_image_shape": (c_int, [c_int, c_int, c_int, c_int, _P, _P, _P]),
    "frcnn_prep_image": (c_int, [_P, c_int, c_int, c_int, _P, c_double, _P, c_int, c_int, c_int, _P]),
    "frcnn_prep_image_batched": (c_int, [_P, c_int, c_int, c_int, c_int, _P, c_double, _P, c_int, c_int, c_int, _P]),
    "frcnn_prep_train_image": (c_int, [_P, c_int, c_int, c_int, c_int, _P, c_double, _P, c_int, c_int, c_int, _P, _P, c_int, _P, _P]),
    "frcnn_jpeg_info": (c_int, [_P, c_size_t, _P]),
    "frcnn_jpeg_coef_bytes": (c_size_t, [c_int, c_int, c_int, c_int, c_int]),
    "frcnn_jpeg_entropy_decode": (c_int, [_P, c_size_t, _P, c_size_t]),
    "frcnn_jpeg_pixels_host": (c_int, [_P, c_int, c_int, c_int, c_int, c_int, _P]),
    "frcnn_jpeg_workspace_bytes": (c_size_t, [c_int, c_int, c_int, c_int, c_int]),
    "frcnn_jpeg_pixels": (c_int, [_P, c_int, c_int, c_int, c_int, c_int, _P, _P, c_size_t, _P]),
    "frcnn_gemm_batched_nt": (c_int, [_P, _P, _P, c_int, c_int, c_int, c_int, _P]),
    "frcnn_winograd_filter_transform": (c_int, [_P, c_int, c_int, _P, c_int, _P]),
    "frcnn_winograd_filter_transform_device": (c_int, [_P, c_int, c_int, c_int, c_int, _P, _P]),
    "frcnn_winograd_input_transform": (c_int, [_P, c_int, c_int, c_int, c_int, c_int, _P, _P]),
    "frcnn_winograd_output_transform": (c_int, [_P, c_int, c_int, c_int, c_int, c_int, _P, c_int, _P, _P]),
    "frcnn_winograd7_filter_transform": (c_int, [_P, c_int, c_int, _P, _P]),
    "frcnn_winograd7_filter_transform_device": (c_int, [_P, c_int, c_int, c_int, _P, _P]),
    "frcnn_winograd7_input_transform": (c_int, [_P, c_int, c_int, _P, _P]),
    "frcnn_winograd7_output_transform": (c_int, [_P, c_int, c_int, _P, c_int, _P, _P]),
    "frcnn_winograd_input_transform_h2": (c_int, [_P, c_int, c_int, c_int, c_int, c_int, _P, _P, _P]),
    "frcnn_winograd_output_transform_h2": (c_int, [_P, c_int, c_int, c_int, c_int, c_int, _P, c_int, _P, _P, _P, _P]),
    "frcnn_winograd7_input_transform_h2": (c_int, [_P, c_int, c_int, _P, _P, _P]),
    "frcnn_winograd7_output_transform_h2": (c_int, [_P, c_int, c_int, _P, c_int, _P, _P, _P, _P]),
    "frcnn_set_tuning": (c_int, [c_int, c_int]),
    "frcnn_pack_filter_hwio": (c_int, [_P, c_int, c_int, c_int, c_int, _P, _P]),
    "frcnn_maxpool_nhwc": (c_int, [_P, c_int, c_int, c_int, c_int, c_int, c_int, c_int, c_int, _P, c_int, c_int, _P]),
    "frcnn_dwconv3x3_nhwc": (c_int, [_P, c_int, c_int, c_int, c_int, _P, _P, _P, c_int, c_int, c_int, c_int, c_int, c_int, _P]),
    "frcnn_dwconv3x3_nhwc_h2": (c_int, [_P, c_int, c_int, c_int, c_int, _P, _P, _P, _P, _P, c_int, c_int, c_int, c_int, c_int, c_int, _P]),
    "frcnn_spatial_mean": (c_int, [_P, c_int, c_int, c_int, _P, _P]),
    "frcnn_softmax_rows": (c_int, [_P, c_int, c_int, c_int, _P, _P]),
    "frcnn_rpn_softmax": (c_int, [_P, c_int, c_int, c_int, _P, _P]),
    "frcnn_copy_cols": (c_int, [_P, c_int, c_int, c_int, c_int, _P, c_int, _P]),
    "frcnn_anchor_target_workspace_bytes": (c_size_t, [c_int, c_int, c_int, c_int]),
    "frcnn_anchor_target_layer": (c_int, [_P, c_int, c_float, c_float, c_int, c_int, c_int, c_int, _P, c_int, c_double, c_double,
                                          c_double, c_longlong, _P, _P, _P, _P, _P, _P, c_size_t, _P]),
    "frcnn_anchor_target_layer_inject": (c_int, [_P, c_int, c_float, c_float, c_int, c_int, c_int, c_int, _P, c_int, c_double, c_double,
                                                 c_double, _P, c_int, _P, _P, _P, _P, _P, _P, c_size_t, _P]),
    "frcnn_proposal_target_layer_inject": (c_int, [_P, _P, c_int, _P, c_int, c_int, c_int, _P, c_int, _P, _P, _P, _P, _P, _P, _P, _P, _P, _P]),
    "frcnn_proposal_target_layer": (c_int, [_P, _P, c_int, _P, c_int, c_int, c_int, c_double, c_double, c_double, c_double, _P, _P,
                                            c_longlong, _P, _P, _P, _P, _P, _P, _P, _P, _P]),
    "frcnn_proposal_target_layer_dn": (c_int, [_P, _P, c_int, _P, _P, c_int, c_int, c_int, c_double, c_double, c_double, c_double, _P, _P,
                                               c_longlong, _P, _P, _P, _P, _P, _P, _P, _P, _P]),
    "frcnn_loss_workspace_bytes": (c_size_t, [c_longlong]),
    "frcnn_softmax_ce_loss": (c_int, [_P, _P, c_int, c_int, c_int, c_int, c_int, _P, _P, _P, c_size_t, _P]),
    "frcnn_smooth_l1_loss": (c_int, [_P, _P, _P, _P, c_longlong, c_float, c_float, _P, _P, _P, c_size_t, _P]),
    "frcnn_transpose_pad": (c_int, [_P, c_int, c_int, _P, c_int, _P]),
    "frcnn_im2col_t": (c_int, [_P, c_int, c_int, c_int, c_int, c_int, c_int, c_int, c_int, c_int, c_int, c_int, _P, c_int, _P]),
    "frcnn_flip_transpose_filter": (c_int, [_P, c_int, c_int, c_int, c_int, _P, _P]),
    "frcnn_conv2d_dgrad_strided": (c_int, [_P, c_int, c_int, c_int, c_int, _P, c_int, c_int, c_int, c_int, c_int, c_int, _P, c_int,
                                           c_int, c_int, _P]),
    "frcnn_conv2d_wgrad_supported": (c_int, [c_int, c_int]),
    "frcnn_conv2d_wgrad_workspace_bytes": (c_size_t, [c_int, c_int, c_int, c_int, c_int, c_int, c_int]),
    "frcnn_conv2d_wgrad": (c_int, [_P, _P, c_int, c_int, c_int, c_int, c_int, c_int, c_int, c_int, c_int, c_int, c_int, c_int, _P, _P,
                                   c_size_t, _P]),
    "frcnn_conv2d_wgrad_set_plan": (None, [c_int, c_int]),
    "frcnn_conv2d_wgrad_h2_workspace_bytes": (c_size_t, [c_int, c_int, c_int, c_int, c_int, c_int, c_int]),
    "frcnn_conv2d_wgrad_h2": (c_int, [_P, _P, c_int, c_int, c_int, c_int, c_int, c_int, c_int, c_int, c_int, c_int, c_int, c_int, _P, _P,
                                      c_size_t, _P]),
    "frcnn_conv2d_wgrad_h2_set_plan": (None, [c_int, c_int]),
    "frcnn_relu_bwd": (c_int, [_P, _P, c_longlong, _P]),
    "frcnn_gemm_x3_pack_bytes": (c_size_t, [c_int, c_int, c_int]),
    "frcnn_gemm_x3_pack": (c_int, [_P, c_int, c_int, c_int, _P, _P]),
    "frcnn_gemm_x3": (c_int, [_P, _P, _P, _P, _P, c_int, c_int, c_int, c_int, c_int, c_int, c_int, _P]),
    "frcnn_h2_planes_bytes": (c_size_t, [c_longlong, c_int]),
    "frcnn_h2_pack_w": (c_int, [_P, c_int, c_int, c_int, _P, _P, _P]),
    "frcnn_h2_split": (c_int, [_P, c_longlong, c_int, _P, _P, _P]),
    "frcnn_gemm_h2": (c_int, [_P, _P, _P, _P, _P, _P, _P, _P, _P, _P, _P, c_int, c_int, c_int, c_int, c_int, c_int, _P]),
    "frcnn_gemm_h2_mean_workspace_bytes": (c_size_t, [c_int, c_int, c_int]),
    "frcnn_gemm_h2_mean": (c_int, [_P, _P, _P, _P, _P, _P, _P, _P, c_int, c_int, c_int, c_int, c_int, c_int, _P, _P, c_size_t, c_int, _P]),
    "frcnn_relu6_bwd": (c_int, [_P, _P, c_longlong, _P]),
    "frcnn_maxpool_bwd": (c_int, [_P, c_int, c_int, c_int, c_int, c_int, c_int, _P, _P, c_int, c_int, _P, _P]),
    "frcnn_dropout": (c_int, [_P, c_longlong, c_ulonglong, c_float, _P, _P]),
    "frcnn_dwconv3x3_dgrad": (c_int, [_P, c_int, c_int, c_int, c_int, _P, _P, c_int, c_int, c_int, c_int, c_int, c_int, _P]),
    "frcnn_dwconv3x3_wgrad_workspace_bytes": (c_size_t, [c_int, c_int, c_int, c_int]),
    "frcnn_dwconv3x3_wgrad": (c_int, [_P, _P, c_int, c_int, c_int, c_int, c_int, c_int, c_int, c_int, c_int, _P, _P, _P, c_size_t, _P]),
    "frcnn_dwconv3x3_refold": (c_int, [_P, _P, c_int, _P, _P]),
    "frcnn_add_strided": (c_int, [_P, c_int, c_int, c_int, c_int, _P, c_int, c_int, c_int, c_int, _P]),
    "frcnn_spatial_mean_bwd": (c_int, [_P, c_int, c_int, c_int, _P, _P]),
    "frcnn_colsum": (c_int, [_P, c_int, c_int, _P, _P]),
    "frcnn_crop_and_resize_bwd": (c_int, [_P, c_int, c_int, c_int, _P, c_int, c_float, c_int, _P, _P]),
    "frcnn_crop_and_resize_bwd_plan": (c_int, [_P, c_int, c_int, c_int, _P, c_int, c_float, c_int, _P, c_size_t, _P]),
    "frcnn_sgd_momentum": (c_int, [_P, _P, _P, _P, _P, c_longlong, c_int, c_float, c_float, c_float, c_float, _P]),
    "frcnn_sgd_desc_bytes": (c_size_t, []),
    "frcnn_sgd_momentum_multi": (c_int, [_P, c_int, c_float, c_float, c_float, _P]),
    "frcnn_sgd_momentum_range": (c_int, [_P, c_int, c_int, c_float, c_float, c_float, _P]),
    "frcnn_sumsq": (c_int, [_P, c_longlong, c_double, _P, c_int, _P, c_size_t, _P]),
    "frcnn_sumsq_multi": (c_int, [_P, _P, c_int, c_double, _P, c_int, _P, c_size_t, _P]),
    "frcnn_summary_limits": (c_int, [_P]),
    "frcnn_summary_stats_workspace_bytes": (c_size_t, [c_int]),
    "frcnn_summary_stats": (c_int, [_P, c_int, _P, _P, c_size_t, _P]),
    "frcnn_graph_begin": (c_int, [_P]),
    "frcnn_graph_end": (c_int, [_P, ctypes.POINTER(c_void_p)]),
    "frcnn_graph_launch": (c_int, [_P, _P]),
    "frcnn_graph_destroy": (c_int, [_P]),
}


class FrcnnHipError(RuntimeError):
    pass


def lib():
    global _lib
    if _lib is None:
        if not os.path.exists(LIB_PATH):
            raise ImportError("libfrcnn_hip.so not built: run `python -c 'import __graft_entry__ as g; g.build()'` "
# ... 30 lines not shown
```

### tf-faster-rcnn_amd/frcnn_hip/ops.py

```python
import ctypes

import numpy as np
import torch

import frcnn_hip as _binding
from . import ACT_NONE, NMS_RULE_CPU, call, lib

_ws_cache = {}
ws_scope = "default"

_scope_stack = [(None, None, None)]


def active_store(owner, default=None):
    o, _, store = _scope_stack[-1]
    return store if store is not None and (owner is None or o is owner) else default


def scope_depth():
    return len(_scope_stack) - 1


class unscoped(object):

# ... 231 lines not shown
    return out


def proposal_layer(rpn_cls_prob, rpn_bbox_pred, im_h, im_w, feat_stride, base_d, pre_nms_topn, post_nms_topn,
                   nms_thresh, rois=None, scores=None, num=None, rule=NMS_RULE_CPU):
    _chk(rpn_cls_prob), _chk(rpn_bbox_pred), _chk(base_d, torch.float64)
    B, H, W, A2 = rpn_cls_prob.shape
    A = A2 // 2
    dev = rpn_cls_prob.device
    rois = _empty((B * post_nms_topn, 5), dtype=torch.float32, device=dev) if rois is None else rois
    scores = _empty((B * post_nms_topn, 1), dtype=torch.float32, device=dev) if scores is None else scores
    num = _zeros((B,), dtype=torch.int32, device=dev) if num is None else num
    nb = lib().frcnn_proposal_batched_workspace_bytes(B, H, W, A, int(pre_nms_topn))
    ws = workspace(nb, dev, "proposal")
    call("frcnn_proposal_layer_batched", _ptr(rpn_cls_prob), _ptr(rpn_bbox_pred), B, float(im_h), float(im_w), H, W, A,
         int(feat_stride), _ptr(base_d), int(pre_nms_topn), int(post_nms_topn), float(nms_thresh), int(rule), _ptr(rois),
         _ptr(scores), _ptr(num), _ptr(ws), ws.numel(), _stream())
    return rois, scores, num


def proposal_layer_tf(rpn_cls_prob, rpn_bbox_pred, im_h, im_w, feat_stride, base_d, post_nms_topn, nms_thresh, rois=None,
                      scores=None, num=None):
    _chk(rpn_cls_prob), _chk(rpn_bbox_pred), _chk(base_d, torch.float64)
    B, H, W, A2 = rpn_cls_prob.shape
    A = A2 // 2
    dev = rpn_cls_prob.device
    rois = _empty((B * post_nms_topn, 5), dtype=torch.float32, device=dev) if rois is None else rois
    scores = _empty((B * post_nms_topn, 1), dtype=torch.float32, device=dev) if scores is None else scores
    num = _zeros((B,), dtype=torch.int32, device=dev) if num is None else num
    nb = lib().frcnn_proposal_batched_workspace_bytes(B, H, W, A, 0)
    ws = workspace(nb, dev, "proposal")
    call("frcnn_proposal_layer_tf_batched", _ptr(rpn_cls_prob), _ptr(rpn_bbox_pred), B, float(im_h), float(im_w), H, W, A,
         int(feat_stride), _ptr(base_d), int(post_nms_topn), float(nms_thresh), _ptr(rois), _ptr(scores), _ptr(num),
         _ptr(ws), ws.numel(), _stream())
    return rois, scores, num


def proposal_top_layer_inds(rpn_cls_prob, rpn_bbox_pred, im_h, im_w, feat_stride, base_d, top_inds, rois=None, scores=None):
    _chk(rpn_cls_prob), _chk(rpn_bbox_pred), _chk(base_d, torch.float64), _chk(top_inds, torch.int32)
    _, H, W, A2 = rpn_cls_prob.shape
    n = top_inds.numel()
    dev = rpn_cls_prob.device
    rois = _empty((n, 5), dtype=torch.float32, device=dev) if rois is None else rois
    scores = _empty((n, 1), dtype=torch.float32, device=dev) if scores is None else scores
    call("frcnn_proposal_top_layer_inds", _ptr(rpn_cls_prob), _ptr(rpn_bbox_pred), float(im_h), float(im_w), H, W, A2 // 2,
         int(feat_stride), _ptr(base_d), _ptr(top_inds), n, _ptr(rois), _ptr(scores), _stream())
    return rois, scores


def proposal_top_layer(rpn_cls_prob, rpn_bbox_pred, im_h, im_w, feat_stride, base_d, rpn_top_n, rois=None, scores=None):
    _chk(rpn_cls_prob), _chk(rpn_bbox_pred), _chk(base_d, torch.float64)
    _, H, W, A2 = rpn_cls_prob.shape
    A = A2 // 2
    dev = rpn_cls_prob.device
    rois = _empty((rpn_top_n, 5), dtype=torch.float32, device=dev) if rois is None else rois
    scores = _empty((rpn_top_n, 1), dtype=torch.float32, device=dev) if scores is None else scores
    nb = lib().frcnn_proposal_workspace_bytes(H, W, A, int(rpn_top_n))
    ws = workspace(nb, dev, "proposal")
    call("frcnn_proposal_top_layer", _ptr(rpn_cls_prob), _ptr(rpn_bbox_pred), float(im_h), float(im_w), H, W, A,
         int(feat_stride), _ptr(base_d), int(rpn_top_n), _ptr(rois), _ptr(scores), _ptr(ws), ws.numel(), _stream())
    return rois, scores


def crop_and_resize(feat, rois, feat_stride, pool, max_pool=False, out=None):
    _chk(feat), _chk(rois)
    H, W, C = feat.shape[-3:]
    N = feat.shape[0] if feat.dim() == 4 else 1
    R = rois.shape[0]
    out = _empty((R, pool, pool, C), dtype=torch.float32, device=feat.device) if out is None else out
    call("frcnn_crop_and_resize_batched", _ptr(feat), N, H, W, C, _ptr(rois), R, float(feat_stride), int(pool),
         1 if max_pool else 0, _ptr(out), _stream())
    return out


def crop_and_resize_bias_act(feat, rois, feat_stride, pool, bias, act, out=None):
    _chk(feat), _chk(rois)
    H, W, C = feat.shape[-3:]
    N = feat.shape[0] if feat.dim() == 4 else 1
    R = rois.shape[0]
    out = _empty((R, pool, pool, C), dtype=torch.float32, device=feat.device) if out is None else out
    call("frcnn_crop_and_resize_bias_act", _ptr(feat), N, H, W, C, _ptr(rois), R, float(feat_stride), int(pool), _ptr(bias),
         int(act), _ptr(out), _stream())
    return out


def detect_post(cls_prob, bbox_pred, rois, num_rois, im_scale, im_h, im_w, nms_thresh=0.3, score_thresh=0.0,
                max_per_image=100, max_out=None, out=None, count=None, batch=1, rule=NMS_RULE_CPU):
    _chk(cls_prob), _chk(rois)
    if bbox_pred is not None:
        _chk(bbox_pred)
    B = int(batch)
    R, C = cls_prob.shape[0] // B, cls_prob.shape[1]
    if cls_prob.shape[0] != B * R or rois.shape[0] != B * R:
        raise ValueError("detect_post: %d rows do not split into %d images" % (cls_prob.shape[0], B))
    dev = cls_prob.device
    max_out = (max_per_image + 28 if max_per_image > 0 else R * (C - 1)) if max_out is None else max_out
    shape = (max_out, 6) if B == 1 else (B, max_out, 6)
    out = _empty(shape, dtype=torch.float32, device=dev) if out is None else out
    count = _zeros((B,), dtype=torch.int32, device=dev) if count is None else count
    if out.dtype != torch.float32 or out.shape[-1] != 6 or out.stride(-1) != 1 or out.stride(-2) != 6 or out.shape[-2] < max_out:
        raise ValueError("detect_post: `out` must be float32 [.., >=max_out, 6] with contiguous images")
    out_stride = out.stride(0) if out.dim() == 3 else 0
    nb = lib().frcnn_detect_post_batched_workspace_bytes(B, R, C)
    ws = workspace(nb, dev, "detect_post")
    call("frcnn_detect_post_batched", _ptr(cls_prob), _ptr(bbox_pred), _ptr(rois), _ptr(num_rois), B, R, C, float(im_scale),
         int(im_h), int(im_w), float(nms_thresh), int(rule), float(score_thresh), int(max_per_image), _ptr(out), _ptr(count),
         int(max_out), int(out_stride), _ptr(ws), ws.numel(), _stream())
    return out, count


def im_detect_boxes(rois, bbox_pred, im_scale, im_h, im_w, num_classes=None):
    _chk(rois)
    if bbox_pred is None:
        R, C4 = rois.shape[0], 4 * int(num_classes)
    else:
        _chk(bbox_pred)
        R, C4 = bbox_pred.shape
    out = _empty((R, C4), dtype=torch.float32, device=rois.device)
    call("frcnn_im_detect_boxes", _ptr(rois), _ptr(bbox_pred), R, C4 // 4, float(im_scale), int(im_h), int(im_w), _ptr(out),
         _stream())
    return out


def pack_filter_hwio(w_hwio, scale=None):
    w = np.ascontiguousarray(w_hwio, dtype=np.float32)
    KH, KW, Cin, Cout = w.shape
    out = np.empty((Cout, KH, KW, Cin), dtype=np.float32)
    sc = None if scale is None else np.ascontiguousarray(scale, dtype=np.float32)
    call("frcnn_pack_filter_hwio", w.ctypes.data_as(ctypes.c_void_p), KH, KW, Cin, Cout,
         None if sc is None else sc.ctypes.data_as(ctypes.c_void_p), out.ctypes.data_as(ctypes.c_void_p))
    return out


def pack_filter_foldw(w_hwio, scale=None):
    w = np.asarray(w_hwio, dtype=np.float32)
    KH, KW, Cin, Cout = w.shape
    assert KW <= 8 and Cin <= 4
    if scale is not None:
        w = w * np.asarray(scale, dtype=np.float32)[None, None, None, :]
    out = np.zeros((Cout, KH, 8, 4), dtype=np.float32)
    out[:, :, :KW, :Cin] = np.transpose(w, (3, 0, 1, 2))
    return out


def conv_out_size(n, k, stride, pad_lo, pad_hi):
    return (n + pad_lo + pad_hi - k) // stride + 1


split_k = True


def conv2d(x, w_packed, bias, KH, KW, stride=1, pad=(0, 0, 0, 0), act=ACT_NONE, residual=None, res_stride=1,
           fold_w=False, out=None, mask=None):
    _chk(x), _chk(w_packed)
    N, H, W, Cin = x.shape
    Cout = w_packed.shape[0]
    OH = conv_out_size(H, KH, stride, pad[0], pad[1])
    OW = conv_out_size(W, KW, stride, pad[2], pad[3])
    out = _empty((N, OH, OW, Cout), dtype=torch.float32, device=x.device) if out is None else out
    RH = RW = 0
    if residual is not None:
        _chk(residual)
        RH, RW = residual.shape[1], residual.shape[2]
    nb = lib().frcnn_conv2d_workspace_bytes(N, OH, OW, Cout, KH, KW, Cin, 1 if fold_w else 0) if split_k else 0
    if mask is not None:
        _chk(mask)
# ... 138 lines not shown
    sc = None if scale is None else np.ascontiguousarray(scale, dtype=np.float32)
    if m == 7:
        out = np.empty((121, Cout, Cin), dtype=np.float32)
        call("frcnn_winograd7_filter_transform", w.ctypes.data_as(ctypes.c_void_p), Cin, Cout,
             None if sc is None else sc.ctypes.data_as(ctypes.c_void_p), out.ctypes.data_as(ctypes.c_void_p))
        return out
    out = np.empty(((m + 2) ** 2, Cout, Cin), dtype=np.float32)
    call("frcnn_winograd_filter_transform", w.ctypes.data_as(ctypes.c_void_p), Cin, Cout,
         None if sc is None else sc.ctypes.data_as(ctypes.c_void_p), int(m), out.ctypes.data_as(ctypes.c_void_p))
    return out


def winograd_filter_transform_device(w_packed, m=4, transpose_flip=False, out=None):
    _chk(w_packed)
    O, kh, kw, C = w_packed.shape
    assert kh == 3 and kw == 3
    G = winograd_points(m)
    shape = (G, C, O) if transpose_flip else (G, O, C)
    out = _empty(shape, dtype=torch.float32, device=w_packed.device) if out is None else out
    assert out.numel() == G * O * C
    if m == 7:
        call("frcnn_winograd7_filter_transform_device", _ptr(w_packed), O, C, 1 if transpose_flip else 0, _ptr(out), _stream())
    else:
        call("frcnn_winograd_filter_transform_device", _ptr(w_packed), O, C, int(m), 1 if transpose_flip else 0, _ptr(out), _stream())
    return out.view(shape)


def winograd_points(m):
    return 121 if m == 7 else (m + 2) ** 2


def winograd_tiles(N, H, W, m):
    if m == 7:
        assert H == 7 and W == 7
        return N
    return N * ((H + m - 1) // m) * ((W + m - 1) // m)


def winograd_input_transform(x, v, m=2):
    _chk(x), _chk(v)
    N, H, W, C = x.shape
    assert v.numel() == winograd_points(m) * winograd_tiles(N, H, W, m) * C
    if m == 7:
        call("frcnn_winograd7_input_transform", _ptr(x), N, C, _ptr(v), _stream())
    else:
        call("frcnn_winograd_input_transform", _ptr(x), N, H, W, C, int(m), _ptr(v), _stream())
    return v


def gemm_batched_nt(x, w, y):
    _chk(x), _chk(w), _chk(y)
    G, M, K = x.shape
    N = w.shape[1]
    assert w.shape == (G, N, K) and y.shape == (G, M, N)
    call("frcnn_gemm_batched_nt", _ptr(x), _ptr(w), _ptr(y), G, M, N, K, _stream())
    return y


def winograd_output_transform(mm, bias, act, out, m=2):
    _chk(mm), _chk(out)
    N, H, W, C = out.shape
    assert mm.numel() == winograd_points(m) * winograd_tiles(N, H, W, m) * C
    if m == 7:
        call("frcnn_winograd7_output_transform", _ptr(mm), N, C, _ptr(bias), int(act), _ptr(out), _stream())
    else:
        call("frcnn_winograd_output_transform", _ptr(mm), N, H, W, C, int(m), _ptr(bias), int(act), _ptr(out), _stream())
    return out


def winograd_output_transform_masked(mm, mask, out, m, out_planes=None):
    _chk(mm), _chk(mask), _chk(out)
    N, H, W, C = out.shape
    assert mm.numel() == winograd_points(m) * winograd_tiles(N, H, W, m) * C and mask.numel() == out.numel()
    if out_planes is not None:
        assert isinstance(out_planes, H2) and out_planes.rows == N * H * W and out_planes.K == C
    pl, inv = (None, None) if out_planes is None else (out_planes.planes, out_planes.inv)
    if m == 7:
        call("frcnn_winograd7_output_transform_masked", _ptr(mm), N, C, _ptr(mask), _ptr(out), _ptr(pl), _ptr(inv), _stream())
    else:
        call("frcnn_winograd_output_transform_masked", _ptr(mm), N, H, W, C, int(m), _ptr(mask), _ptr(out), _ptr(pl), _ptr(inv), _stream())
    return out


def conv3x3_winograd(x, u, bias, act=ACT_NONE, out=None, v_buf=None, m_buf=None, u_planes=None, v_planes=None, mask=None, out_planes=None):
    N, H, W, Cin = x.shape
    G, Cout = u.shape[0], u.shape[1]
    m = {16: 2, 36: 4, 121: 7}[G]
    T = winograd_tiles(N, H, W, m)
    dev = x.device
    mm = _empty((G, T, Cout), dtype=torch.float32, device=dev) if m_buf is None else m_buf
    out = _empty((N, H, W, Cout), dtype=torch.float32, device=dev) if out is None else out
    if u_planes is not None:
        v_planes = H2.empty(G * T, Cin, dev) if v_planes is None else v_planes
        winograd_input_transform_h2(x, v_planes, m)
        gemm_h2(v_planes, u_planes, G, T, Cout, Cin, out=mm.view(G * T, Cout))
    else:
        v = _empty((G, T, Cin), dtype=torch.float32, device=dev) if v_buf is None else v_buf
        winograd_input_transform(x, v, m)
        gemm_batched_nt(v, u, mm)
    if mask is not None:
        assert bias is None and act == ACT_NONE
        return winograd_output_transform_masked(mm, mask, out, m, out_planes)
    if out_planes is not None:
        winograd_output_transform_h2(mm, bias, act, tuple(out.shape), m, out_planes, out)
        return out
    return winograd_output_transform(mm, bias, act, out, m)


def maxpool(x, k, stride, pad=(0, 0, 0, 0), out=None):
    _chk(x)
    N, H, W, C = x.shape
    OH = conv_out_size(H, k, stride, pad[0], pad[1])
    OW = conv_out_size(W, k, stride, pad[2], pad[3])
    out = _empty((N, OH, OW, C), dtype=torch.float32, device=x.device) if out is None else out
    call("frcnn_maxpool_nhwc", _ptr(x), N, H, W, C, int(k), int(stride), int(pad[0]), int(pad[2]), _ptr(out), OH, OW,
         _stream())
    return out


def dwconv3x3(x, w, bias, stride=1, pad=(1, 1, 1, 1), act=ACT_NONE, out=None, out_planes=None, want_f32=True):
    _chk(x), _chk(w)
    N, H, W, C = x.shape
    OH = conv_out_size(H, 3, stride, pad[0], pad[1])
    OW = conv_out_size(W, 3, stride, pad[2], pad[3])
    if out_planes is None:
        out = _empty((N, OH, OW, C), dtype=torch.float32, device=x.device) if out is None else out
        call("frcnn_dwconv3x3_nhwc", _ptr(x), N, H, W, C, _ptr(w), _ptr(bias), _ptr(out), OH, OW, int(stride),
             int(pad[0]), int(pad[2]), int(act), _stream())
        return out
    assert isinstance(out_planes, H2) and out_planes.rows == N * OH * OW and out_planes.K == C
    if want_f32 and out is None:
        out = _empty((N, OH, OW, C), dtype=torch.float32, device=x.device)
    call("frcnn_dwconv3x3_nhwc_h2", _ptr(x), N, H, W, C, _ptr(w), _ptr(bias), _ptr(out if want_f32 else None), _ptr(out_planes.planes),
         _ptr(out_planes.inv), OH, OW, int(stride), int(pad[0]), int(pad[2]), int(act), _stream())
    return out if want_f32 else None


def spatial_mean(x, out=None):
    _chk(x)
    N, C = x.shape[0], x.shape[-1]
    HW = x.numel() // (N * C)
    out = _empty((N, C), dtype=torch.float32, device=x.device) if out is None else out
    call("frcnn_spatial_mean", _ptr(x), N, HW, C, _ptr(out), _stream())
    return out


def softmax_rows(x, C=None, out=None):
    _chk(x)
    R, ld = x.shape
    C = ld if C is None else C
    out = _empty((R, C), dtype=torch.float32, device=x.device) if out is None else out
    call("frcnn_softmax_rows", _ptr(x), R, C, ld, _ptr(out), _stream())
    return out


def rpn_softmax(score, A, out=None):
    _chk(score)
    N, H, W, ld = score.shape
    out = _empty((N, H, W, 2 * A), dtype=torch.float32, device=score.device) if out is None else out
    call("frcnn_rpn_softmax", _ptr(score), N * H * W, A, ld, _ptr(out), _stream())
    return out


def copy_cols(src, col0, cols, out=None):
    _chk(src)
    ld = src.shape[-1]
    R = src.numel() // ld
    out = _empty(tuple(src.shape[:-1]) + (cols,), dtype=torch.float32, device=src.device) if out is None else out
    call("frcnn_copy_cols", _ptr(src), R, ld, int(col0), int(cols), _ptr(out), cols, _stream())
    return out


def _host_doubles(values):
    a = np.ascontiguousarray(values, dtype=np.float64)
    if _binding.recorder is not None:
        _binding.recorder.keep.append(a)
    return a, a.ctypes.data_as(ctypes.c_void_p)
# ... 470 lines not shown
```

### tf-faster-rcnn_amd/frcnn_hip/runtime.py

```python
import collections
import os
import time

import numpy as np
import torch

from . import ops


class VarSpec(object):
    __slots__ = ("shape", "init", "arg")

    def __init__(self, shape, init, arg=None):
        self.shape, self.init, self.arg = tuple(int(s) for s in shape), init, arg


class VariableStore(object):
    prepared = None

    def __init__(self, seed=3):
        self.variables = collections.OrderedDict()
        self.packed = {}
        self.x3 = {}
        self.h2 = {}
# ... 296 lines not shown
        return self.scopes.pop(key, None) is not None

    def _store(self):
        return ops.active_store(self, self.buffers)

    def find_buf(self, name, shape, dtype=torch.float32):
        key = (name, tuple(shape), dtype)
        for st in [ops.active_store(self, {})] + list(reversed(self.scopes.values())) + [self.buffers]:
            if key in st:
                return st[key]
        raise KeyError(key)

    def scope_bytes(self, key=None):
        def size(v):
            if torch.is_tensor(v):
                return v.numel() * v.element_size()
            if isinstance(v, (tuple, list)):
                return sum(size(x) for x in v)
            return sum(size(getattr(v, a)) for a in ("planes", "inv") if hasattr(v, a))
        stores = [self.scopes[key]] if key is not None else list(self.scopes.values())
        return sum(size(v) for st in stores for v in st.values())

    def buf(self, name, shape, dtype=torch.float32, zero=False):
        key = (name, tuple(shape), dtype)
        top = ops._scope_stack[-1]
        store = top[2] if top[0] is self else self.buffers
        t = store.get(key)
        if t is None:
            t = store[key] = (torch.zeros if zero else torch.empty)(tuple(shape), dtype=dtype, device=self.device)
            if self.poison_new_buffers and not zero:
                t.view(torch.uint8).fill_(0xFF)
        return t

    def x3_planes(self, w):
        key = (w.data_ptr(), tuple(w.shape))
        self.prepared.wait_planes()
        ent = self.x3.get(key)
        if ent is None:
            ent = (ops.gemm_x3_pack(w), w)
            self.x3[key] = ent
            self.derived_gen += 1
        return ent[0]

    def wino_refresh(self):
        n = 0
        for key, val in list(self.packed.items()):
            if isinstance(key, tuple) and key and key[0] == "wino":
                u = val[0]
                info = self.conv_info.get(key[1])
                if info is not None and info["w"].dim() == 4 and info["w"].shape[1] == 3:
                    ops.winograd_filter_transform_device(info["w"], key[3], False, out=u)
                    n += 1
        return n

    def x3_refresh(self):
        for planes, w in self.x3.values():
            ops.gemm_x3_pack(w, planes)

    def h2_channel_spread(self, scope):
        got = self.h2_spread.get(scope)
        if got is None:
            w = np.abs(self.variables[scope + "/weights"].astype(np.float64))
            if w.ndim == 2:
                w = w[None, None]
            if (scope + "/BatchNorm/gamma") in self.variables:
                v = self.variables
                w = w * np.abs(v[scope + "/BatchNorm/gamma"].astype(np.float64) / np.sqrt(v[scope + "/BatchNorm/moving_variance"].astype(np.float64) + 1e-5))
            per_k = w.max(axis=(0, 1, 3))
            top = float(per_k.max())
            nz = per_k[per_k > 0]
            got = self.h2_spread[scope] = (float(nz.min()) / top) if (top > 0 and nz.size) else 1.0
        return got

    def h2_planes(self, w):
        key = (w.data_ptr(), tuple(w.shape))
        self.prepared.wait_planes()
        ent = self.h2.get(key)
        if ent is None:
            ent = (ops.h2_pack_w(w), w)
            self.h2[key] = ent
            self.derived_gen += 1
        return ent[0]

    def h2_refresh(self):
        for packed, w in self.h2.values():
            ops.h2_pack_w(w, packed)

    def h2_buf(self, name, rows, K):
        key = ("h2", name, int(rows), int(K))
        store = ops.active_store(self, self.buffers)
        t = store.get(key)
        if t is None:
            t = store[key] = ops.H2.empty(rows, K, self.device)
        return t

    def buf_pair(self, name, N, K):
        key = ("h2w", name, int(N), int(K))
        t = self.buffers.get(key)
        if t is None:
            t = self.buffers[key] = (torch.empty(int(ops.lib().frcnn_h2_planes_bytes(int(N), int(K))), dtype=torch.uint8, device=self.device),
                                     torch.empty((1, int(N)), dtype=torch.float32, device=self.device))
        return t

    def mark(self, tag, flops, fn, nbytes=0):
        self.flops_last_forward += flops
        if flops and self.flops_by_pipe is not None:
            pipe = "h2" if tag.startswith("conv:h2:") else "x3" if tag.startswith("conv:x3:") else "f32"
            self.flops_by_pipe[pipe] = self.flops_by_pipe.get(pipe, 0) + flops
        if self.profile is None:
            return fn()
        e0, e1 = torch.cuda.Event(enable_timing=True), torch.cuda.Event(enable_timing=True)
        e0.record()
        r = fn()
        e1.record()
        self.profile.append((tag, flops, e0, e1, nbytes))
        return r

    def synchronize(self):
        torch.cuda.current_stream(self.device).synchronize()

    def close(self):
        for d in (self.graphs, self.scopes, self.scope_group, self.buffers, self.packed, self.x3, self.h2):
            d.clear()


class Timer(object):

    def __init__(self):
        self.total_time = 0.
        self.calls = 0
        self.start_time = 0.
        self.diff = 0.
        self.average_time = 0.

    def tic(self):
        self.start_time = time.time()

    def toc(self, average=True):
        self.diff = time.time() - self.start_time
        self.total_time += self.diff
        self.calls += 1
        self.average_time = self.total_time / self.calls
        return self.average_time if average else self.diff
```

### tf-faster-rcnn_amd/lib/model/config.py

```python
import ast
import os
import os.path as osp

import numpy as np


class AttrDict(dict):

    def __init__(self, d=None, **kw):
        super().__init__()
        for k, v in dict(d or {}, **kw).items():
            self[k] = v

    def __setitem__(self, k, v):
        if isinstance(v, dict) and not isinstance(v, AttrDict):
            v = AttrDict(v)
        super().__setitem__(k, v)

    def __getattr__(self, k):
        try:
            return self[k]
        except KeyError:
            raise AttributeError(k)

    __setattr__ = __setitem__


_TRAIN = dict(
    LEARNING_RATE=0.001, MOMENTUM=0.9, WEIGHT_DECAY=0.0001, GAMMA=0.1, STEPSIZE=[30000], DISPLAY=10,
    DOUBLE_BIAS=True, TRUNCATED=False, BIAS_DECAY=False, USE_GT=False, ASPECT_GROUPING=False,
    SNAPSHOT_KEPT=3, SUMMARY_INTERVAL=180, SCALES=(600,), MAX_SIZE=1000, IMS_PER_BATCH=1, BATCH_SIZE=128,
    FG_FRACTION=0.25, FG_THRESH=0.5, BG_THRESH_HI=0.5, BG_THRESH_LO=0.1, USE_FLIPPED=True, BBOX_REG=True,
    BBOX_THRESH=0.5, SNAPSHOT_ITERS=5000, SNAPSHOT_PREFIX='res101_faster_rcnn', BBOX_NORMALIZE_TARGETS=True,
    BBOX_INSIDE_WEIGHTS=(1.0, 1.0, 1.0, 1.0), BBOX_NORMALIZE_TARGETS_PRECOMPUTED=True,
    BBOX_NORMALIZE_MEANS=(0.0, 0.0, 0.0, 0.0), BBOX_NORMALIZE_STDS=(0.1, 0.1, 0.2, 0.2), PROPOSAL_METHOD='gt',
    HAS_RPN=True, RPN_POSITIVE_OVERLAP=0.7, RPN_NEGATIVE_OVERLAP=0.3, RPN_CLOBBER_POSITIVES=False,
    RPN_FG_FRACTION=0.5, RPN_BATCHSIZE=256, RPN_NMS_THRESH=0.7, RPN_PRE_NMS_TOP_N=12000,
    RPN_POST_NMS_TOP_N=2000, RPN_BBOX_INSIDE_WEIGHTS=(1.0, 1.0, 1.0, 1.0), RPN_POSITIVE_WEIGHT=-1.0,
    USE_ALL_GT=True)

_TEST = dict(
    SCALES=(600,), MAX_SIZE=1000, NMS=0.3, SVM=False, BBOX_REG=True, HAS_RPN=False, PROPOSAL_METHOD='gt',
    RPN_NMS_THRESH=0.7, RPN_PRE_NMS_TOP_N=6000, RPN_POST_NMS_TOP_N=300, MODE='nms', RPN_TOP_N=5000)

__C = AttrDict(
    TRAIN=_TRAIN, TEST=_TEST,
    RESNET=dict(MAX_POOL=False, FIXED_BLOCKS=1),
    MOBILENET=dict(REGU_DEPTH=False, FIXED_LAYERS=5, WEIGHT_DECAY=0.00004, DEPTH_MULTIPLIER=1.),
    PIXEL_MEANS=np.array([[[102.9801, 115.9465, 122.7717]]]), RNG_SEED=3,
    ROOT_DIR=osp.abspath(osp.join(osp.dirname(__file__), '..', '..')),
    MATLAB='matlab', EXP_DIR='default', USE_GPU_NMS=True, USE_E2E_TF=False, POOLING_MODE='crop', POOLING_SIZE=7,
    ANCHOR_SCALES=[8, 16, 32], ANCHOR_RATIOS=[0.5, 1, 2], RPN_CHANNELS=512,
    HIP=dict(WINOGRAD=True, WINOGRAD_MIN_CIN=64, WINOGRAD_M=4, WINOGRAD_F2_SCOPES=("block1", "block2"), WINOGRAD_DIRECT_SCOPES=(),
             WINOGRAD_TRAIN=True, WINOGRAD_DGRAD=True,
             WINOGRAD_7X7=True, FUSE_TAIL_MEAN=True, MFMA_X3=True,
             MFMA_H2=True, H2_LAZY_SPLIT=True, H2_MIN_TILES=150, H2_TRAIN_MIN_TILES=320, H2_TRUNK_PLANES=True, H2_TILE_CFG=-1,
             X3_TILE_CFG=-1, H2_TRAIN=True, WGRAD_STREAM=2, WGRAD_TN=True, WGRAD_H2=True, PREP_STREAM=True, TRAIN_REPLAY=True, TRAIN_PICK_STREAMS=6,
             GRAPH_CACHE_SHAPES=4, TRAIN_CACHE_SHAPES=16, JPEG_DEVICE=False, TEST_BATCH_IMAGES=1))
__C.DATA_DIR = osp.abspath(osp.join(__C.ROOT_DIR, 'data'))
cfg = __C


def get_output_dir(imdb, weights_filename):
    outdir = osp.abspath(osp.join(__C.ROOT_DIR, 'output', __C.EXP_DIR, imdb.name))
    outdir = osp.join(outdir, 'default' if weights_filename is None else weights_filename)
    os.makedirs(outdir, exist_ok=True)
    return outdir


def get_output_tb_dir(imdb, weights_filename):
    outdir = osp.abspath(osp.join(__C.ROOT_DIR, 'tensorboard', __C.EXP_DIR, imdb.name))
    outdir = osp.join(outdir, 'default' if weights_filename is None else weights_filename)
    os.makedirs(outdir, exist_ok=True)
    return outdir


_NULLABLE_KEYS = ("H2_TRAIN_MIN_TILES",)


def _merge_a_into_b(a, b):
    if not isinstance(a, dict):
        return
    for k, v in a.items():
        if k not in b:
            raise KeyError('{} is not a valid config key'.format(k))
        old = b[k]
        if type(old) is not type(v) and not (isinstance(old, dict) and isinstance(v, dict)):
            if isinstance(old, np.ndarray):
                v = np.array(v, dtype=old.dtype)
            elif isinstance(old, tuple) and isinstance(v, list):
                v = tuple(v)
            elif isinstance(old, list) and isinstance(v, tuple):
                v = list(v)
            elif k in _NULLABLE_KEYS and (v is None or old is None) and isinstance(old if v is None else v, int):
                pass
            else:
                raise ValueError('Type mismatch ({} vs. {}) for config key: {}'.format(type(old), type(v), k))
        if isinstance(v, dict):
            try:
                _merge_a_into_b(v, b[k])
            except Exception:
                print('Error under config key: {}'.format(k))
                raise
        else:
            b[k] = v


def cfg_from_file(filename):
    import yaml
    with open(filename, 'r') as f:
        _merge_a_into_b(AttrDict(yaml.safe_load(f) or {}), __C)


def cfg_from_list(cfg_list):
    assert len(cfg_list) % 2 == 0
    for k, v in zip(cfg_list[0::2], cfg_list[1::2]):
        path = k.split('.')
        d = __C
        for sub in path[:-1]:
            assert sub in d
            d = d[sub]
        leaf = path[-1]
        assert leaf in d
        try:
            value = ast.literal_eval(v)
        except Exception:
            value = v
        old = d[leaf]
        if isinstance(old, tuple) and isinstance(value, list):
            value = tuple(value)
        if isinstance(old, list) and isinstance(value, tuple):
            value = list(value)
        nullable = leaf in _NULLABLE_KEYS and (value is None or old is None) and isinstance(old if value is None else value, int)
        assert nullable or type(value) == type(old), 'type {} does not match original type {}'.format(type(value), type(old))
        d[leaf] = value
```

### tf-faster-rcnn_amd/lib/nets/network.py

```python
import collections

import numpy as np
import torch

from frcnn_hip import ACT_NONE, ACT_RELU, NMS_RULE_CPU, NMS_RULE_GPU, ops
from frcnn_hip.runtime import VarSpec
from model.config import cfg


class Network(object):
    def __init__(self):
        self._predictions = {}
        self._losses = {}
        self._anchor_targets = {}
        self._proposal_targets = {}
        self._layers = {}
        self._act_summaries = []
        self._variables_to_fix = {}
        self._feat_stride = [16, ]
        self._scope = "network"
        self._sess = None
        self._image = None
        self._im_info = None
        self._var_specs = collections.OrderedDict()
# ... 79 lines not shown
            if residual is not None and residual.data_ptr() in self._f32_missing:
                res = self._h2_of[residual.data_ptr()]
            tcfg = int(cfg.HIP.H2_TILE_CFG)
            sess.mark("conv:h2:" + scope, flops, lambda: ops.gemm_h2(xp, wp, 1, M, Cout, Cin, b, res, act, out=y, out_planes=yp,
                                                                      want_f32=False, cfg=tcfg),
                      nbytes=4 * M * Cin + 4 * w.numel() + (4 * out.numel() if y is not None else 0)
                      + (4 * out.numel() if yp is not None else 0) + (4 * out.numel() if residual is not None else 0))
            self._wrote(out, yp, y is not None)
        elif plain and self._x3_eligible(M, Cout, Cin, 1):
            self._need_f32(x), self._need_f32(residual)
            planes = sess.x3_planes(w)
            xc = int(cfg.HIP.X3_TILE_CFG)
            sess.mark("conv:x3:" + scope, flops, lambda: ops.gemm_x3(x, planes, 1, M, Cout, Cin, b, residual, act, out=out, cfg=xc),
                      nbytes=4 * (x.numel() + out.numel() + (out.numel() if residual is not None else 0)) + 6 * w.numel())
            self._wrote(out)
        else:
            self._need_f32(x), self._need_f32(residual)
            sess.mark("conv:" + scope, flops,
                      lambda: ops.conv2d(x, w, b, k, k, stride, pad, act, residual, res_stride, fold_w, out=out),
                      nbytes=4 * (x.numel() + w.numel() + out.numel() + (out.numel() if residual is not None else 0)))
            self._wrote(out)
        if self._mode == "TRAIN":
            self._tape.append(dict(kind="conv", scope=scope, x=x, y=out, k=k, stride=stride, pad=tuple(pad), act=act,
                                   residual=residual, res_stride=res_stride))
            if self.trainable_scope(scope) or x.data_ptr() in self._requires_grad:
                self._requires_grad.add(out.data_ptr())
            if residual is not None and residual.data_ptr() in self._requires_grad:
                self._requires_grad.add(out.data_ptr())
        return out

    H2_MIN_CHANNEL_RATIO = 2.0 ** -18

    def _h2_eligible(self, M, N, K, G, scope=None):
        rows = G * M
        if scope is not None and self._mode == "TEST" and self._sess.h2_channel_spread(scope) < self.H2_MIN_CHANNEL_RATIO:
            return False
        return (bool(cfg.HIP.MFMA_H2) and (self._mode == "TEST" or bool(cfg.HIP.H2_TRAIN)) and K % 128 == 0 and N % 128 == 0
                and ((self._plan_rows(M) + 127) // 128) * (N // 128) * G >= self._h2_min_tiles()
                and 4 * rows * K < (1 << 32) and 4 * N * K < (1 << 32) and M * N < (1 << 29))

    @staticmethod
    def h2_min_tiles(mode):
        if mode == "TRAIN" and cfg.HIP.H2_TRAIN_MIN_TILES is not None:
            return int(cfg.HIP.H2_TRAIN_MIN_TILES)
        return int(cfg.HIP.H2_MIN_TILES)

    def _h2_min_tiles(self):
        return self.h2_min_tiles(self._mode)

    def _h2_input(self, x):
        xp = self._h2_of.get(x.data_ptr())
        if xp is None and cfg.HIP.H2_LAZY_SPLIT:
            self._need_f32(x)
            K = x.shape[-1]
            xp = self._sess.h2_buf(self._tag + "/split@%x" % x.data_ptr(), x.numel() // K, K)
            self._sess.mark("op:h2_split", 0, lambda: ops.h2_split(x, out=xp), nbytes=8 * x.numel())
            self._h2_of[x.data_ptr()] = xp
        return xp

    def _wrote(self, t, planes=None, f32=True):
        k = t.data_ptr()
        if planes is None:
            self._h2_of.pop(k, None)
        else:
            self._h2_of[k] = planes
        (self._f32_missing.discard if f32 else self._f32_missing.add)(k)
        return t

    def _need_f32(self, x):
        if x is not None and x.data_ptr() in self._f32_missing:
            raise RuntimeError("graph construction error: a float32 consumer reads a tensor that was emitted as operand planes only")

    def _x3_eligible(self, M, N, K, G):
        return (bool(cfg.HIP.MFMA_X3) and self._mode == "TEST" and N % 64 == 0 and K % 32 == 0
                and ((self._plan_rows(M) + 127) // 128) * ((N + 127) // 128) * G >= 150 and M * N < (1 << 31) and N * K < (1 << 28))

    @staticmethod
    def _winograd_scheme(scope, H, W):
        if any(tok in scope for tok in cfg.HIP.WINOGRAD_F2_SCOPES):
            return 2
        m = int(cfg.HIP.WINOGRAD_M)
        return 7 if (m == 4 and H == 7 and W == 7 and cfg.HIP.WINOGRAD_7X7) else m

    def _conv_winograd(self, x, scope, act, bn_eps, emit_h2=False, want_f32=True):
        sess = self._sess
        self._need_f32(x)
        N, H, W, Cin = x.shape
        m = self._winograd_scheme(scope, H, W)
        u, b = sess.winograd_params(scope, bn_eps=bn_eps, m=m)
        G, Cout = u.shape[0], u.shape[1]
        T = ops.winograd_tiles(N, H, W, m)
        mm = sess.buf(self._tag + "/wino_m", (G, T, Cout))
        out = sess.buf(self._tag + "/" + scope, (N, H, W, Cout))
        flops = 2 * G * T * Cout * Cin
        if self._h2_eligible(T, Cout, Cin, G, scope):
            vp, wp = sess.h2_buf(self._tag + "/wino_v", G * T, Cin), sess.h2_planes(u)
            sess.mark("op:wino_in", 0, lambda: ops.winograd_input_transform_h2(x, vp, m), nbytes=4 * (x.numel() + G * T * Cin))
            tcfg = int(cfg.HIP.H2_TILE_CFG)
            sess.mark("conv:h2:" + scope, flops, lambda: ops.gemm_h2(vp, wp, G, T, Cout, Cin, out=mm, cfg=tcfg),
                      nbytes=4 * (G * T * Cin + mm.numel()) + 4 * u.numel())
        else:
            v = sess.buf(self._tag + "/wino_v", (G, T, Cin))
            sess.mark("op:wino_in", 0, lambda: ops.winograd_input_transform(x, v, m), nbytes=4 * (x.numel() + v.numel()))
            if self._x3_eligible(T, Cout, Cin, G):
                planes = sess.x3_planes(u)
                xc = int(cfg.HIP.X3_TILE_CFG)
                sess.mark("conv:x3:" + scope, flops, lambda: ops.gemm_x3(v, planes, G, T, Cout, Cin, out=mm, cfg=xc),
                          nbytes=4 * (v.numel() + mm.numel()) + 6 * u.numel())
            else:
                sess.mark("conv:" + scope, flops, lambda: ops.gemm_batched_nt(v, u, mm), nbytes=4 * (v.numel() + u.numel() + mm.numel()))
        if emit_h2 and cfg.HIP.MFMA_H2 and Cout % 128 == 0:
            yp = sess.h2_buf(self._tag + "/" + scope, N * H * W, Cout)
            y = out if want_f32 else None
            sess.mark("op:wino_out", 0, lambda: ops.winograd_output_transform_h2(mm, b, act, (N, H, W, Cout), m, yp, y),
                      nbytes=4 * (mm.numel() + out.numel() * (2 if want_f32 else 1)))
            self._wrote(out, yp, y is not None)
        else:
            sess.mark("op:wino_out", 0, lambda: ops.winograd_output_transform(mm, b, act, out, m), nbytes=4 * (mm.numel() + out.numel()))
            self._wrote(out)
        return out

    def _conv1x1_mean(self, x, scope, group_rows, act=ACT_RELU, bn_eps=None, residual=None, name="fc7"):
        sess = self._sess
        w, b = sess.conv_params(scope, bn_eps=bn_eps)
        Cin, Cout = x.shape[-1], w.shape[0]
        rows = x.numel() // Cin
        G = max(1, self._plan_batch)
        assert rows % G == 0 and (rows // G) % group_rows == 0
        M = rows // G
        out = sess.buf(self._tag + "/" + name, (rows // group_rows, Cout))
        xp, wp = self._h2_of[x.data_ptr()], sess.h2_planes(w)
        res = residual
        if residual is not None and residual.data_ptr() in self._f32_missing:
            res = self._h2_of[residual.data_ptr()]
        tcfg = int(cfg.HIP.H2_TILE_CFG)
        sess.mark("conv:h2:" + scope, 2 * rows * Cout * Cin, lambda: ops.gemm_h2_mean(xp, wp, G, M, Cout, Cin, b, res, act, group_rows, out=out, cfg=tcfg),
                  nbytes=4 * (rows * Cin + w.numel() + out.numel() + (rows * Cout if residual is not None else 0)))
        return self._wrote(out)

    def _mean_fusable(self, rows, cout, cin, scope, group_rows=1):
        G = max(1, self._plan_batch)
        return (bool(cfg.HIP.FUSE_TAIL_MEAN) and self._mode == "TEST" and rows % G == 0 and (rows // G) % max(1, int(group_rows)) == 0
                and self._h2_eligible(rows, cout, cin, 1, scope)
                and bool(cfg.HIP.H2_LAZY_SPLIT or cfg.HIP.WINOGRAD))

    _rgb_first_conv = None

    def get_variables_to_restore(self, variables, var_keep_dic):
        skip = set(self._variables_to_fix_names())
        self._variables_to_fix = {}
        keep = []
        for name in variables:
            if name in skip:
                self._variables_to_fix[name] = True
                continue
            if name in var_keep_dic:
                keep.append(name)
        return keep

    def _variables_to_fix_names(self):
        return [] if self._rgb_first_conv is None else [self._scope + self._rgb_first_conv + "/weights"]

    def fix_variables(self, sess, pretrained_model):
        from frcnn_hip.tensor_bundle import open_checkpoint
        reader = open_checkpoint(pretrained_model)
        fixed = {}
        for name in self._variables_to_fix_names():
            fixed[name] = self._fix_one(name, reader.get_tensor(name))
        sess.load_variables(fixed)
        sess.conv_info.clear()
        return sorted(fixed)

    def _fix_one(self, name, value):
        return np.ascontiguousarray(value[:, :, ::-1, :])

    def trainable_scope(self, scope):
        return True

    def _reshape_layer(self, bottom, num_dim, name):
        raise NotImplementedError("folded into frcnn_rpn_softmax (network.py:68-78 only served the pair softmax)")
# ... 212 lines not shown
        with self._plan_context(self, is_training):
            return self._build_network_impl(is_training)

    def _build_network_impl(self, is_training=True):
        self._tape = []
        self._requires_grad = set()
        self._act_summaries = []
        self._h2_of, self._f32_missing = {}, set()
        net_conv = self._image_to_head(is_training)
        self._anchor_component()
        fused = self._fuse_tail_entry and not is_training and hasattr(self, "_fused_tail_entry")
        rois = self._region_proposal(net_conv, is_training)
        if cfg.POOLING_MODE != "crop":
            raise NotImplementedError
        if fused:
            fc7 = self._fused_tail_entry(net_conv, rois)
        else:
            pool5 = self._crop_pool_layer(net_conv, rois, "pool5")
            self._layers["pool5"] = pool5
            fc7 = self._head_to_tail(pool5, is_training)
        self._layers["fc7"] = fc7
        cls_prob, bbox_pred = self._region_classification(fc7, is_training)
        return rois, cls_prob, bbox_pred

    _trainable_on_device = False

    @staticmethod
    def _check_supported_cfg(mode):
        t = cfg.TRAIN
        fixed = [("POOLING_MODE", cfg.POOLING_MODE, "crop")]
        bad = ["%s = %r (only %r is implemented)" % (k, v, want) for k, v, want in fixed if v != want]
        if float(t.RPN_POSITIVE_WEIGHT) >= 0 and not (0.0 < float(t.RPN_POSITIVE_WEIGHT) < 1.0):
            bad.append("TRAIN.RPN_POSITIVE_WEIGHT = %r (the reference asserts 0 < p < 1, anchor_target_layer.py:103-104)" % (t.RPN_POSITIVE_WEIGHT,))
        if bad:
            raise NotImplementedError("unsupported configuration for the HIP path: " + "; ".join(bad))

    def create_architecture(self, mode, num_classes, tag=None, anchor_scales=(8, 16, 32), anchor_ratios=(0.5, 1, 2)):
        assert tag is not None
        self._check_supported_cfg(mode)
        if mode == "TRAIN" and not self._trainable_on_device:
            raise NotImplementedError("%s: no reverse sweep for this network's TRAIN graph; TEST mode works" % type(self).__name__)
        self._tag = tag
        self._num_classes = num_classes
        self._mode = mode
        self._anchor_scales = tuple(anchor_scales)
        self._num_scales = len(anchor_scales)
        self._anchor_ratios = tuple(anchor_ratios)
        self._num_ratios = len(anchor_ratios)
        self._num_anchors = self._num_scales * self._num_ratios
        A = self._num_anchors
        self._var_specs.clear()
        self._declare_backbone()
        hc = self._head_channels()
        self._declare_conv_bias(self._scope + "/rpn_conv/3x3", 3, 3, hc, cfg.RPN_CHANNELS, 0.01)
        self._declare_conv_bias(self._scope + "/rpn_cls_score", 1, 1, cfg.RPN_CHANNELS, 2 * A, 0.01)
        self._declare_conv_bias(self._scope + "/rpn_bbox_pred", 1, 1, cfg.RPN_CHANNELS, 4 * A, 0.01)
        tc = self._tail_channels()
        self._var(self._scope + "/cls_score/weights", (tc, num_classes), "normal", 0.01)
        self._var(self._scope + "/cls_score/biases", (num_classes,), "zeros")
        self._var(self._scope + "/bbox_pred/weights", (tc, 4 * num_classes), "normal", 0.001)
        self._var(self._scope + "/bbox_pred/biases", (4 * num_classes,), "zeros")
        names = ["rois", "rpn_cls_score", "rpn_cls_prob", "rpn_bbox_pred", "cls_score", "cls_prob", "bbox_pred"]
        return {k: k for k in names}

    def _stage_image(self, sess, image, im_info=None):
        if isinstance(image, np.ndarray):
            image = torch.from_numpy(np.ascontiguousarray(image, dtype=np.float32))
        B, H, W, C = image.shape
        if im_info is None:
            buf = sess.buf(self._tag + "/image", (B, H, W, 4), zero=True)
        else:
            with self.shape_scope(sess, (B, H, W, 4), im_info):
                buf = sess.buf(self._tag + "/image", (B, H, W, 4), zero=True)
        buf[..., :C].copy_(image, non_blocking=True)
        return buf

    def graph_key(self, image_shape, im_info):
        c = cfg[self._mode]
        return (self._tag, self._scope, self._num_classes, self._anchor_scales, self._anchor_ratios, bool(cfg.RESNET.MAX_POOL),
                bool(cfg.USE_GPU_NMS), tuple(int(v) for v in image_shape), (float(im_info[0]), float(im_info[1])), self._mode, cfg.TEST.MODE, self._fuse_tail_entry,
                c.RPN_PRE_NMS_TOP_N, c.RPN_POST_NMS_TOP_N, c.RPN_NMS_THRESH, cfg.TEST.RPN_TOP_N, cfg.POOLING_SIZE,
                bool(cfg.HIP.WINOGRAD), int(cfg.HIP.WINOGRAD_MIN_CIN), int(cfg.HIP.WINOGRAD_M), tuple(cfg.HIP.WINOGRAD_F2_SCOPES),
                tuple(cfg.HIP.WINOGRAD_DIRECT_SCOPES), bool(cfg.HIP.WINOGRAD_7X7), bool(cfg.HIP.FUSE_TAIL_MEAN), bool(cfg.HIP.MFMA_X3), bool(cfg.USE_E2E_TF),
                bool(cfg.HIP.MFMA_H2), bool(cfg.HIP.H2_LAZY_SPLIT), int(cfg.HIP.H2_MIN_TILES), bool(cfg.HIP.H2_TRUNK_PLANES), int(cfg.HIP.H2_TILE_CFG), int(cfg.HIP.X3_TILE_CFG), bool(cfg.HIP.H2_TRAIN))

    def shape_scope(self, sess, image_shape, im_info):
        return sess.shape_scope(self.graph_key(image_shape, im_info), group=("graphs", self._tag), cap=int(cfg.HIP.GRAPH_CACHE_SHAPES))

    def forward_device(self, sess, image_d, im_info, use_graph=True):
        self._sess = sess
        self._image = image_d
        self._im_info = (float(im_info[0]), float(im_info[1]), float(im_info[2]))
        sess.prepared.wait_planes()
        ops.ws_scope = self._tag
        key = self.graph_key(image_d.shape, self._im_info)
        cur = torch.cuda.current_stream(sess.device)
        with self.shape_scope(sess, image_d.shape, self._im_info):
            if not use_graph or sess.profile is not None:
                sess.flops_last_forward = 0
                self._build_network(self._mode == "TRAIN")
                return self._predictions
            if key not in sess.graphs:
                with torch.cuda.stream(sess.stream):
                    sess.stream.wait_stream(cur)
                    sess.flops_last_forward = 0
                    self._build_network(False)
                    sess.stream.synchronize()
                    flops = sess.flops_last_forward
                    g = ops.Graph().capture(lambda: self._build_network(False))
                    sess.stream.synchronize()
                sess.graphs[key] = (g, dict(self._predictions), self._num_rois, flops, self._rois_per_image, image_d)
            g, preds, num, flops, per, captured = sess.graphs[key]
            self._predictions, self._num_rois, sess.flops_last_forward, self._rois_per_image = dict(preds), num, flops, per
            if captured.data_ptr() != image_d.data_ptr():
                captured.copy_(image_d, non_blocking=True)
            g.launch()
        return self._predictions

    def extract_head(self, sess, image):
        self._sess = sess
        sess.prepared.wait_planes()
        shape = (int(image.shape[0]), int(image.shape[1]), int(image.shape[2]), 4)
        with sess.shape_scope(("extract_head", self._tag, shape), group=("head", self._tag), cap=int(cfg.HIP.GRAPH_CACHE_SHAPES)):
            self._image = self._stage_image(sess, image)
            self._h2_of, self._f32_missing = {}, set()
            ops.ws_scope = self._tag
            with self._plan_context(self, False):
                feat = self._image_to_head(False)
            return feat.cpu().numpy()

    def test_image(self, sess, image, im_info):
        img = self._stage_image(sess, image, im_info)
        p = self.forward_device(sess, img, im_info)
        assert img.shape[0] == 1, "test_image keeps the reference's single-image contract (network.py:388); use detect_device for batches"
        n = p["rois"].shape[0] if self._num_rois is None else int(self._num_rois.item())
        return (p["cls_score"][:n].cpu().numpy(), p["cls_prob"][:n].cpu().numpy(), p["bbox_pred"][:n].cpu().numpy(),
                p["rois"][:n].cpu().numpy())

    def _stage_train_inputs(self, sess, blobs):
        self._sess = sess
        info = blobs["im_info"]
        self._im_info = (float(info[0]), float(info[1]), float(info[2]))
        if "data" not in blobs:
            im = blobs["image"]
            im_scale, OH, OW = self._train_prep_shape(blobs)
            dev = sess.device
            G = int(blobs["boxes"].shape[0])
            cap = max(self.TRAIN_MAX_GT, (G + 63) // 64 * 64)
            self._image = sess.buf(self._tag + "/image", (1, OH, OW, 4), zero=True)
            buf = sess.buf(self._tag + "/gt_boxes", (cap, 5), zero=True)
            im_d = (im if torch.is_tensor(im) else torch.from_numpy(np.ascontiguousarray(im))).to(dev, non_blocking=True)
            boxes_d = torch.from_numpy(np.ascontiguousarray(blobs["boxes"], dtype=np.uint16)).to(dev, non_blocking=True) if G else None
            classes_d = torch.from_numpy(np.ascontiguousarray(blobs["gt_classes"], dtype=np.int32)).to(dev, non_blocking=True) if G else None
            ops.prep_train_image(im_d, bool(blobs["flipped"]), cfg.PIXEL_MEANS, im_scale, (OH, OW), out=self._image, out_c=4,
                                 boxes=boxes_d, classes=classes_d, gt_out=buf)
            self._gt_boxes = buf[:G]
            return
        self._image = self._stage_image(sess, blobs["data"])
        gt = blobs["gt_boxes"]
        gt = gt if torch.is_tensor(gt) else torch.from_numpy(np.ascontiguousarray(gt, dtype=np.float32))
        G = int(gt.shape[0])
        cap = max(self.TRAIN_MAX_GT, (G + 63) // 64 * 64)
        buf = sess.buf(self._tag + "/gt_boxes", (cap, 5), zero=True)
        buf[:G].copy_(gt, non_blocking=True)
        self._gt_boxes = buf[:G]

    @staticmethod
# ... 265 lines not shown
```

### tf-faster-rcnn_amd/lib/nets/resnet_v1.py

```python
from frcnn_hip import ACT_NONE, ACT_RELU, ops
from model.config import cfg
from nets.network import Network

BN_EPS = 1e-5


def _same_pad(k, stride):
    total = k - 1
    beg = total // 2
    return (beg, total - beg, beg, total - beg)


class resnetv1(Network):
    _rgb_first_conv = "/conv1"
    _trainable_on_device = True
    def __init__(self, num_layers=50):
        Network.__init__(self)
        self._feat_stride = [16, ]
        self._feat_compress = [1. / float(self._feat_stride[0]), ]
        self._num_layers = num_layers
        self._scope = 'resnet_v1_%d' % num_layers
        self._decide_blocks()

    def _decide_blocks(self):
# ... 12 lines not shown
            depth = base * 4
            for u in range(1, n_units + 1):
                p = "%s/%s/unit_%d/bottleneck_v1" % (s, name, u)
                if cin != depth:
                    self._declare_conv_bn(p + "/shortcut", 1, 1, cin, depth)
                self._declare_conv_bn(p + "/conv1", 1, 1, cin, base)
                self._declare_conv_bn(p + "/conv2", 3, 3, base, base)
                self._declare_conv_bn(p + "/conv3", 1, 1, base, depth, residual_branch_end=True)
                cin = depth

    def _head_channels(self):
        return self._blocks[2][1] * 4

    def _tail_channels(self):
        return self._blocks[3][1] * 4

    def _bottleneck(self, x, prefix, base, stride, mean_rows=0, emit_out=True, f32_out=True):
        depth = base * 4
        cin = x.shape[-1]
        if cin != depth:
            shortcut = self._conv(x, prefix + "/shortcut", 1, stride, act=ACT_NONE, bn_eps=BN_EPS)
            res_stride = 1
        else:
            shortcut, res_stride = x, stride
        r = self._conv(x, prefix + "/conv1", 1, 1, act=ACT_RELU, bn_eps=BN_EPS)
        pad = (1, 1, 1, 1) if stride == 1 else _same_pad(3, stride)
        N, H, W, _ = r.shape
        M3 = N * ops.conv_out_size(H, 3, stride, pad[0], pad[1]) * ops.conv_out_size(W, 3, stride, pad[2], pad[3])
        if mean_rows and res_stride == 1 and stride == 1 and self._mean_fusable(M3, depth, base, prefix + "/conv3", mean_rows):
            r = self._conv(r, prefix + "/conv2", 3, stride, pad, act=ACT_RELU, bn_eps=BN_EPS, emit_h2=True, want_f32=False)
            if self._h2_input(r) is not None:
                return self._conv1x1_mean(r, prefix + "/conv3", mean_rows, act=ACT_RELU, bn_eps=BN_EPS, residual=shortcut)
            x = self._conv(r, prefix + "/conv3", 1, 1, act=ACT_RELU, bn_eps=BN_EPS, residual=shortcut, res_stride=1)
            out = self._sess.buf(self._tag + "/fc7", (x.shape[0], x.shape[-1]))
            return self._sess.mark("op:spatial_mean", 0, lambda: ops.spatial_mean(x, out=out), nbytes=4 * (x.numel() + out.numel()))
        c3_h2 = res_stride == 1 and self._h2_eligible(M3, depth, base, 1, prefix + "/conv3")
        r = self._conv(r, prefix + "/conv2", 3, stride, pad, act=ACT_RELU, bn_eps=BN_EPS, emit_h2=c3_h2, want_f32=not c3_h2)
        return self._conv(r, prefix + "/conv3", 1, 1, act=ACT_RELU, bn_eps=BN_EPS, residual=shortcut, res_stride=res_stride,
                          emit_h2=emit_out, want_f32=f32_out)

    def _trunk_planes_only(self, rows, base, next_stride, next_prefix=None):
        depth = 4 * base
        return (bool(cfg.HIP.H2_TRUNK_PLANES) and next_stride == 1
                and self._h2_eligible(rows, base, depth, 1, None if next_prefix is None else next_prefix + "/conv1")
                and self._h2_eligible(rows, depth, base, 1, None if next_prefix is None else next_prefix + "/conv3"))

    def _run_blocks(self, x, blocks, emit_last=True):
        for bi, (name, base, n_units, stride) in enumerate(blocks):
            for u in range(1, n_units + 1):
                s_u = stride if u == n_units else 1
                N, H, W, _ = x.shape
                rows = N * ops.conv_out_size(H, 3, s_u, 1, 1) * ops.conv_out_size(W, 3, s_u, 1, 1) if s_u > 1 else N * H * W
                planes_only = u < n_units and self._trunk_planes_only(rows, base, stride if u + 1 == n_units else 1,
                                                                       "%s/%s/unit_%d/bottleneck_v1" % (self._scope, name, u + 1))
                x = self._bottleneck(x, "%s/%s/unit_%d/bottleneck_v1" % (self._scope, name, u), base, s_u,
                                     emit_out=emit_last or u < n_units or bi + 1 < len(blocks), f32_out=not planes_only)
        return x

    def _crop_pool_layer(self, bottom, rois, name):
        return self._crop_pool(bottom, rois, name, max_pool=bool(cfg.RESNET.MAX_POOL))

    def _build_base(self):
        net = self._conv(self._image, self._scope + "/conv1", 7, 2, _same_pad(7, 2), act=ACT_RELU, bn_eps=BN_EPS,
                         fold_w=True, real_cin=3)
        N, H, W, C = net.shape
        out = self._sess.buf(self._tag + "/pool1", (N, ops.conv_out_size(H, 3, 2, 1, 1), ops.conv_out_size(W, 3, 2, 1, 1), C))
        self._sess.mark("op:maxpool", 0, lambda: ops.maxpool(net, 3, 2, (1, 1, 1, 1), out=out), nbytes=4 * (net.numel() + out.numel()))
        return self._wrote(out)

    def _image_to_head(self, is_training, reuse=None):
        assert (0 <= cfg.RESNET.FIXED_BLOCKS <= 3)
        net_conv = self._run_blocks(self._build_base(), self._blocks[0:3])
        self._act_summaries.append(net_conv)
        self._layers['head'] = net_conv
        return net_conv

    def _fused_tail_maps(self, net_conv):
        name = self._blocks[-1][0]
        prefix = "%s/%s/unit_1/bottleneck_v1" % (self._scope, name)
        sc_map = self._conv(net_conv, prefix + "/shortcut", 1, 1, act=ACT_NONE, bn_eps=BN_EPS, no_bias=True)
        c1_map = self._conv(net_conv, prefix + "/conv1", 1, 1, act=ACT_NONE, bn_eps=BN_EPS, no_bias=True)
        return sc_map, c1_map

    def _fused_tail_entry(self, net_conv, rois):
        sess, P = self._sess, cfg.POOLING_SIZE
        name, base, n_units, stride = self._blocks[-1]
        prefix = "%s/%s/unit_1/bottleneck_v1" % (self._scope, name)
        R = rois.shape[0]
        sc_map, c1_map = self._fused_tail_maps(net_conv)
        b_sc = sess.conv_info[prefix + "/shortcut"]["b"]
        b_c1 = sess.conv_info[prefix + "/conv1"]["b"]
        fs = float(self._feat_stride[0])
        sc_out = sess.buf(self._tag + "/" + prefix + "/shortcut_crop", (R, P, P, sc_map.shape[-1]))
        c1_out = sess.buf(self._tag + "/" + prefix + "/conv1_crop", (R, P, P, c1_map.shape[-1]))
        shortcut = self._crop_images(sc_map, rois, sc_out, bias=b_sc, act=ACT_NONE)
        r = self._crop_images(c1_map, rois, c1_out, bias=b_c1, act=ACT_RELU)
        c3_h2 = self._h2_eligible(R * P * P, 4 * base, base, 1, prefix + "/conv3")
        r = self._conv(r, prefix + "/conv2", 3, 1, (1, 1, 1, 1), act=ACT_RELU, bn_eps=BN_EPS, emit_h2=c3_h2, want_f32=not c3_h2)
        x = self._conv(r, prefix + "/conv3", 1, 1, act=ACT_RELU, bn_eps=BN_EPS, residual=shortcut, res_stride=1, emit_h2=n_units >= 2,
                       want_f32=not (n_units >= 2 and self._trunk_planes_only(R * P * P, base, stride if n_units == 2 else 1,
                                                                              "%s/%s/unit_2/bottleneck_v1" % (self._scope, name))))
        fused = stride == 1 and n_units >= 2 and self._mean_fusable(R * P * P, 4 * base, base, "%s/%s/unit_%d/bottleneck_v1/conv3" % (self._scope, name, n_units), P * P)
        for u in range(2, n_units + 1):
            x = self._bottleneck(x, "%s/%s/unit_%d/bottleneck_v1" % (self._scope, name, u), base, stride if u == n_units else 1,
                                 mean_rows=P * P if (fused and u == n_units) else 0, emit_out=u < n_units,
                                 f32_out=not (u < n_units and self._trunk_planes_only(R * P * P, base, stride if u + 1 == n_units else 1,
                                                                                      "%s/%s/unit_%d/bottleneck_v1" % (self._scope, name, u + 1))))
        if fused:
            return x
        out = sess.buf(self._tag + "/fc7", (x.shape[0], x.shape[-1]))
        return sess.mark("op:spatial_mean", 0, lambda: ops.spatial_mean(x, out=out), nbytes=4 * (x.numel() + out.numel()))

    def _head_to_tail(self, pool5, is_training, reuse=None):
        name, base, n_units, stride = self._blocks[-1]
        if stride == 1 and self._mean_fusable(pool5.shape[0] * pool5.shape[1] * pool5.shape[2], 4 * base, base,
                                              "%s/%s/unit_%d/bottleneck_v1/conv3" % (self._scope, name, n_units), pool5.shape[1] * pool5.shape[2]):
            x = pool5
            hw = pool5.shape[1] * pool5.shape[2]
            for u in range(1, n_units + 1):
                x = self._bottleneck(x, "%s/%s/unit_%d/bottleneck_v1" % (self._scope, name, u), base, 1, mean_rows=hw if u == n_units else 0)
            return x
        fc7 = self._run_blocks(pool5, self._blocks[-1:], emit_last=False)
        out = self._sess.buf(self._tag + "/fc7", (fc7.shape[0], fc7.shape[-1]))
        res = self._sess.mark("op:spatial_mean", 0, lambda: ops.spatial_mean(fc7, out=out), nbytes=4 * (fc7.numel() + out.numel()))
        if self._mode == "TRAIN":
            self._tape.append(dict(kind="mean", x=fc7, y=res, name=self._scope + "/fc7_mean"))
            if fc7.data_ptr() in self._requires_grad:
                self._requires_grad.add(res.data_ptr())
        return res

    def trainable_scope(self, scope):
        fixed = ["/conv1"] + ["/block%d/" % b for b in range(1, cfg.RESNET.FIXED_BLOCKS + 1)]
        tail = scope[len(self._scope):]
        return not any(tail.startswith(f) for f in fixed)
```

Baseline: 527.3.

## Fuse tail-entry shortcut/conv1 GEMMs and crop into winograd7 input transform

At test time the block-4 entry shortcut and conv1 1x1 convolutions are merged into one concatenated h2 GEMM producing a single map. A new kernel then crops the conv1 channels per ROI, applies bias and ReLU, and writes the Winograd 7x7 input-transform planes directly, while a companion kernel crops the shortcut. This removes a separate GEMM launch, the intermediate conv1 crop tensor and the standalone winograd input transform. It also restricts the double-epilogue GEMM config to K<512. The gain comes with more code paths and a large-register fused kernel.

```diff
diff --git a/include/frcnn_hip.h b/include/frcnn_hip.h
--- a/include/frcnn_hip.h
+++ b/include/frcnn_hip.h
@@ -169,6 +169,9 @@
 int frcnn_winograd7_input_transform_h2(const float* x_d, int R, int C, void* v_planes_d, float* v_inv_d, void* stream);
 int frcnn_winograd7_output_transform_h2(const float* m_d, int R, int C, const float* bias_d, int act, float* y_d, void* y_planes_d,
                                         float* y_inv_d, void* stream);
+int frcnn_crop_tail_entry(const float* feat_d, int N, int H, int W, int C_sc, int C_c1, const float* rois_d, int R, float feat_stride,
+                          int pool, const float* bias_sc_d, const float* bias_c1_d, float* sc_out_d, void* v_planes_d, float* v_inv_d,
+                          void* stream);
 int frcnn_pack_filter_hwio(const float* w_hwio, int KH, int KW, int Cin, int Cout, const float* scale, float* out);
 int frcnn_maxpool_nhwc(const float* x_d, int N, int H, int W, int C, int k, int stride, int pad_top,
                        int pad_left, float* y_d, int OH, int OW, void* stream);
diff --git a/tf-faster-rcnn_amd/csrc/crop_common.h b/tf-faster-rcnn_amd/csrc/crop_common.h
--- /dev/null
+++ b/tf-faster-rcnn_amd/csrc/crop_common.h
@@ -0,0 +1,103 @@
+#pragma once
+#include "common.h"
+
+__device__ __forceinline__ float4 lerp4(const float4 a, const float4 b, float t) {
+  return make_float4(a.x + (b.x - a.x) * t, a.y + (b.y - a.y) * t, a.z + (b.z - a.z) * t, a.w + (b.w - a.w) * t);
+}
+__device__ __forceinline__ float2 lerp4(const float2 a, const float2 b, float t) {
+  return make_float2(a.x + (b.x - a.x) * t, a.y + (b.y - a.y) * t);
+}
+__device__ __forceinline__ float4 max4(const float4 a, const float4 b) {
+  return make_float4(fmaxf(a.x, b.x), fmaxf(a.y, b.y), fmaxf(a.z, b.z), fmaxf(a.w, b.w));
+}
+__device__ __forceinline__ void crop_zero(float4& v) { v = make_float4(0, 0, 0, 0); }
+__device__ __forceinline__ void crop_zero(float2& v) { v = make_float2(0, 0); }
+
+__device__ __forceinline__ float crop_coord(float a1, int n, float step, int g) { return a1 * (float)(n - 1) + (float)g * step; }
+
+template <typename V>
+__device__ __forceinline__ V crop_sample(const V* __restrict__ feat, int H, int W, int CV, int cv, float y1, float x1, float hs, float ws,
+                                         int gy, int gx) {
+  const float in_y = crop_coord(y1, H, hs, gy);
+  const float in_x = crop_coord(x1, W, ws, gx);
+  if (in_y < 0 || in_y > (float)(H - 1) || in_x < 0 || in_x > (float)(W - 1)) {
+    V zero;
+    crop_zero(zero);
+    return zero;
+  }
+  const int top = (int)floorf(in_y), bot = (int)ceilf(in_y);
+  const int left = (int)floorf(in_x), right = (int)ceilf(in_x);
+  const float ly = in_y - (float)top, lx = in_x - (float)left;
+  const V tl = feat[((size_t)top * W + left) * CV + cv], tr = feat[((size_t)top * W + right) * CV + cv];
+  const V bl = feat[((size_t)bot * W + left) * CV + cv], br = feat[((size_t)bot * W + right) * CV + cv];
+  return lerp4(lerp4(tl, tr, lx), lerp4(bl, br, lx), ly);
+}
+
+__device__ __forceinline__ bool crop_axis(float a1, int n, float step, int g, int& lo, int& hi, float& frac) {
+  float in = crop_coord(a1, n, step, g);
+  const bool inside = !((in < 0) | (in > (float)(n - 1)));
+  in = inside ? in : 0.f;
+  lo = (int)floorf(in);
+  hi = (int)ceilf(in);
+  frac = in - (float)lo;
+  return inside;
+}
+
+template <bool MAX2, int ITEMS>
+__device__ __forceinline__ void crop_roi_slab(int blk, const float4* __restrict__ feat_all, int NIMG, int H, int W, int FC4, int C4, int nslab,
+                                              const float* __restrict__ rois, float stride, int pool, const float4* __restrict__ bias, int act,
+                                              float4* __restrict__ out) {
+  const int slab = blk % nslab, r = blk / nslab;
+  const int SC4 = C4 / nslab, c40 = slab * SC4;
+  const float height = ((float)H - 1.0f) * stride, width = ((float)W - 1.0f) * stride;
+  const float* roi = rois + 5 * (size_t)r;
+  const int img = (int)roi[0];
+  float4* obase = out + (size_t)r * pool * pool * C4;
+  const int total = pool * pool * SC4;
+  if (img < 0 || img >= NIMG) {
+    for (int t = threadIdx.x; t < total; t += 256) obase[(size_t)(t / SC4) * C4 + c40 + t % SC4] = make_float4(0, 0, 0, 0);
+    return;
+  }
+  const float4* feat = feat_all + (size_t)img * H * W * FC4;
+  const float x1 = roi[1] / width, y1 = roi[2] / height, x2 = roi[3] / width, y2 = roi[4] / height;
+  const int P = MAX2 ? 2 * pool : pool;
+  const float hs = (y2 - y1) * (float)(H - 1) / (float)(P - 1);
+  const float ws = (x2 - x1) * (float)(W - 1) / (float)(P - 1);
+  for (int t0 = threadIdx.x; t0 < total; t0 += 256 * ITEMS) {
+    float4 v[ITEMS];
+#pragma unroll
+    for (int k = 0; k < ITEMS; ++k) {
+      const int t = t0 + k * 256;
+      if (t >= total) { v[k] = make_float4(0, 0, 0, 0); continue; }
+      const int pix = t / SC4, c4 = c40 + t % SC4;
+      const int py = pix / pool, px = pix - py * pool;
+      if (MAX2) {
+        v[k] = crop_sample(feat, H, W, FC4, c4, y1, x1, hs, ws, 2 * py, 2 * px);
+        v[k] = max4(v[k], crop_sample(feat, H, W, FC4, c4, y1, x1, hs, ws, 2 * py, 2 * px + 1));
+        v[k] = max4(v[k], crop_sample(feat, H, W, FC4, c4, y1, x1, hs, ws, 2 * py + 1, 2 * px));
+        v[k] = max4(v[k], crop_sample(feat, H, W, FC4, c4, y1, x1, hs, ws, 2 * py + 1, 2 * px + 1));
+      } else {
+        v[k] = crop_sample(feat, H, W, FC4, c4, y1, x1, hs, ws, py, px);
+      }
+    }
+#pragma unroll
+    for (int k = 0; k < ITEMS; ++k) {
+      const int t = t0 + k * 256;
+      if (t >= total) continue;
+      const int pix = t / SC4, c4 = c40 + t % SC4;
+      float4 o = v[k];
+      if (bias) {
+        const float4 bv = bias[c4];
+        o.x += bv.x; o.y += bv.y; o.z += bv.z; o.w += bv.w;
+      }
+      if (act == FRCNN_ACT_RELU) o = act_relu(o);
+      obase[(size_t)pix * C4 + c4] = o;
+    }
+  }
+}
+
+static inline int crop_roi_slabs(int C4) {
+  int nslab = (C4 % 8 == 0 && C4 / 8 >= 16) ? 8 : 1;
+  if (nslab == 8 && C4 / 8 < 32) nslab = 4;
+  return nslab;
+}
diff --git a/tf-faster-rcnn_amd/csrc/detect_kernels.hip b/tf-faster-rcnn_amd/csrc/detect_kernels.hip
--- a/tf-faster-rcnn_amd/csrc/detect_kernels.hip
+++ b/tf-faster-rcnn_amd/csrc/detect_kernels.hip
@@ -1,4 +1,5 @@
 #include "common.h"
+#include "crop_common.h"
 
 extern "C" int frcnn_generate_anchors(int base_size, const double* ratios, int n_ratios, const double* scales,
                                       int n_scales, double* out_base) {
@@ -817,26 +818,6 @@
                                          nms_thresh, rois_d, scores_d, num_d, ws, ws_bytes, stream);
 }
 
-__device__ __forceinline__ float4 lerp4(const float4 a, const float4 b, float t) {
-  return make_float4(a.x + (b.x - a.x) * t, a.y + (b.y - a.y) * t, a.z + (b.z - a.z) * t, a.w + (b.w - a.w) * t);
-}
-__device__ __forceinline__ float4 max4(const float4 a, const float4 b) {
-  return make_float4(fmaxf(a.x, b.x), fmaxf(a.y, b.y), fmaxf(a.z, b.z), fmaxf(a.w, b.w));
-}
-
-__device__ __forceinline__ float4 crop_sample(const float4* __restrict__ feat, int H, int W, int C4, int c4, float y1,
-                                              float x1, float hs, float ws, int gy, int gx) {
-  const float in_y = y1 * (float)(H - 1) + (float)gy * hs;
-  const float in_x = x1 * (float)(W - 1) + (float)gx * ws;
-  if (in_y < 0 || in_y > (float)(H - 1) || in_x < 0 || in_x > (float)(W - 1)) return make_float4(0, 0, 0, 0);
-  const int top = (int)floorf(in_y), bot = (int)ceilf(in_y);
-  const int left = (int)floorf(in_x), right = (int)ceilf(in_x);
-  const float ly = in_y - (float)top, lx = in_x - (float)left;
-  const float4 tl = feat[((size_t)top * W + left) * C4 + c4], tr = feat[((size_t)top * W + right) * C4 + c4];
-  const float4 bl = feat[((size_t)bot * W + left) * C4 + c4], br = feat[((size_t)bot * W + right) * C4 + c4];
-  return lerp4(lerp4(tl, tr, lx), lerp4(bl, br, lx), ly);
-}
-
 template <bool MAX2>
 __global__ __launch_bounds__(256) void k_crop_and_resize(const float4* __restrict__ feat_all, int NIMG, int H, int W, int C4,
                                                          int nslab, const float* __restrict__ rois, float stride, int pool,
@@ -881,53 +862,7 @@
 __global__ __launch_bounds__(256) void k_crop_and_resize_roi(const float4* __restrict__ feat_all, int NIMG, int H, int W, int C4,
                                                              int nslab, const float* __restrict__ rois, float stride, int pool,
                                                              const float4* __restrict__ bias, int act, float4* __restrict__ out) {
-  const int slab = blockIdx.x % nslab, r = blockIdx.x / nslab;
-  const int SC4 = C4 / nslab, c40 = slab * SC4;
-  const float height = ((float)H - 1.0f) * stride, width = ((float)W - 1.0f) * stride;
-  const float* roi = rois + 5 * (size_t)r;
-  const int img = (int)roi[0];
-  float4* obase = out + (size_t)r * pool * pool * C4;
-  const int total = pool * pool * SC4;
-  if (img < 0 || img >= NIMG) {
-    for (int t = threadIdx.x; t < total; t += 256) obase[(size_t)(t / SC4) * C4 + c40 + t % SC4] = make_float4(0, 0, 0, 0);
-    return;
-  }
-  const float4* feat = feat_all + (size_t)img * H * W * C4;
-  const float x1 = roi[1] / width, y1 = roi[2] / height, x2 = roi[3] / width, y2 = roi[4] / height;
-  const int P = MAX2 ? 2 * pool : pool;
-  const float hs = (y2 - y1) * (float)(H - 1) / (float)(P - 1);
-  const float ws = (x2 - x1) * (float)(W - 1) / (float)(P - 1);
-  for (int t0 = threadIdx.x; t0 < total; t0 += 256 * ITEMS) {
-    float4 v[ITEMS];
-#pragma unroll
-    for (int k = 0; k < ITEMS; ++k) {
-      const int t = t0 + k * 256;
-      if (t >= total) { v[k] = make_float4(0, 0, 0, 0); continue; }
-      const int pix = t / SC4, c4 = c40 + t % SC4;
-      const int py = pix / pool, px = pix - py * pool;
-      if (MAX2) {
-        v[k] = crop_sample(feat, H, W, C4, c4, y1, x1, hs, ws, 2 * py, 2 * px);
-        v[k] = max4(v[k], crop_sample(feat, H, W, C4, c4, y1, x1, hs, ws, 2 * py, 2 * px + 1));
-        v[k] = max4(v[k], crop_sample(feat, H, W, C4, c4, y1, x1, hs, ws, 2 * py + 1, 2 * px));
-        v[k] = max4(v[k], crop_sample(feat, H, W, C4, c4, y1, x1, hs, ws, 2 * py + 1, 2 * px + 1));
-      } else {
-        v[k] = crop_sample(feat, H, W, C4, c4, y1, x1, hs, ws, py, px);
-      }
-    }
-#pragma unroll
-    for (int k = 0; k < ITEMS; ++k) {
-      const int t = t0 + k * 256;
-      if (t >= total) continue;
-      const int pix = t / SC4, c4 = c40 + t % SC4;
-      float4 o = v[k];
-      if (bias) {
-        const float4 bv = bias[c4];
-        o.x += bv.x; o.y += bv.y; o.z += bv.z; o.w += bv.w;
-      }
-      if (act == FRCNN_ACT_RELU) o = act_relu(o);
-      obase[(size_t)pix * C4 + c4] = o;
-    }
-  }
+  crop_roi_slab<MAX2, ITEMS>((int)blockIdx.x, feat_all, NIMG, H, W, C4, C4, nslab, rois, stride, pool, bias, act, out);
 }
 
 static thread_local int g_crop_slabs = -1;
@@ -941,7 +876,7 @@
   hipStream_t st = (hipStream_t)stream;
   const int C4 = C / 4;
   int nslab = (C4 % 8 == 0 && C4 / 8 >= 16) ? 8 : 1;
-  if (g_crop_form == 0 && nslab == 8 && C4 / 8 < 32) nslab = 4;
+  if (g_crop_form == 0) nslab = crop_roi_slabs(C4);
   if (g_crop_slabs > 0 && C4 % g_crop_slabs == 0) nslab = g_crop_slabs;
   const long long blocks = (long long)R * pool * nslab;
   if (blocks >= (1ll << 31)) return FRCNN_E_UNSUPPORTED;
diff --git a/tf-faster-rcnn_amd/csrc/gemm_h2.hip b/tf-faster-rcnn_amd/csrc/gemm_h2.hip
--- a/tf-faster-rcnn_amd/csrc/gemm_h2.hip
+++ b/tf-faster-rcnn_amd/csrc/gemm_h2.hip
@@ -1134,7 +1134,7 @@
     const int pp_cfg = (cfg == -3 || cfg == -4 || (cfg == -6 && K < FRCNN_H2_PP_MIN_K)) ? 34 : 21;
     const bool pp = K >= pp_min_k && mt256 * 256 * 100 <= (long long)M * 104 && mt256 * (N / 128) * G >= 256;
     const bool tiny = (long long)((M + 127) / 128) * (N / 128) * G < 150;
-    const bool de = cfg != -2 && cfg != -7 && !p.mean_part && !p.mask && ((p.resp && p.yp && !p.y) || cfg == -8);
+    const bool de = cfg != -2 && cfg != -7 && !p.mean_part && !p.mask && ((p.resp && p.yp && !p.y && K < 512) || cfg == -8);
     cfg = pp ? pp_cfg : tiny ? (cfg == -2 ? 12 : (de && cfg == -8) ? 41 : 33) : (cfg == -2 ? 9 : de ? 40 : 31);
   }
   if (p.mean_part && (cfg == 40 || cfg == 41)) cfg = cfg == 40 ? 31 : 33;
diff --git a/tf-faster-rcnn_amd/csrc/winograd7.hip b/tf-faster-rcnn_amd/csrc/winograd7.hip
--- a/tf-faster-rcnn_amd/csrc/winograd7.hip
+++ b/tf-faster-rcnn_amd/csrc/winograd7.hip
@@ -1,4 +1,5 @@
 #include "h2_common.h"
+#include "crop_common.h"
 
 namespace w7 {
 constexpr float BT[11][9] = {
@@ -55,6 +56,33 @@
 };
 
 template <bool H2>
+__device__ __forceinline__ void wino7_input_body(const float2 (&d)[7][7], int r, int R, int c2, int C2, const Wino7Sink<H2>& V) {
+#pragma unroll
+  for (int xi = 0; xi < 11; ++xi) {
+    float2 t[7];
+#pragma unroll
+    for (int j = 0; j < 7; ++j) {
+      bool first = true;
+      t[j] = make_float2(0.f, 0.f);
+#pragma unroll
+      for (int i = 0; i < 7; ++i) acc_term(t[j], first, w7::BT[xi][i + 1], d[i][j]);
+    }
+    float2 o[11];
+    size_t rw[11];
+#pragma unroll
+    for (int nu = 0; nu < 11; ++nu) {
+      bool first = true;
+      float2 v = make_float2(0.f, 0.f);
+#pragma unroll
+      for (int j = 0; j < 7; ++j) acc_term(v, first, w7::BT[nu][j + 1], t[j]);
+      o[nu] = v;
+      rw[nu] = (size_t)(xi * 11 + nu) * R + r;
+    }
+    V.template putn<11>(rw, o, c2, C2);
+  }
+}
+
+template <bool H2>
 __global__ void __launch_bounds__(256) k_wino7_input(const float2* __restrict__ x, int R, int C2, const Wino7Sink<H2> V) {
   const long long id = (long long)blockIdx.x * blockDim.x + threadIdx.x;
   if (id >= (long long)R * C2) return;
@@ -66,29 +94,72 @@
   for (int i = 0; i < 7; ++i)
 #pragma unroll
     for (int j = 0; j < 7; ++j) d[i][j] = src[(size_t)(i * 7 + j) * C2];
-#pragma unroll
-  for (int xi = 0; xi < 11; ++xi) {
-    float2 t[7];
-#pragma unroll
-    for (int j = 0; j < 7; ++j) {
-      bool first = true;
-      t[j] = make_float2(0.f, 0.f);
-#pragma unroll
-      for (int i = 0; i < 7; ++i) acc_term(t[j], first, w7::BT[xi][i + 1], d[i][j]);
-    }
-    float2 o[11];
-    size_t rw[11];
-#pragma unroll
-    for (int nu = 0; nu < 11; ++nu) {
-      bool first = true;
-      float2 v = make_float2(0.f, 0.f);
-#pragma unroll
-      for (int j = 0; j < 7; ++j) acc_term(v, first, w7::BT[nu][j + 1], t[j]);
-      o[nu] = v;
-      rw[nu] = (size_t)(xi * 11 + nu) * R + r;
-    }
-    V.template putn<11>(rw, o, c2, C2);
-  }
+  wino7_input_body<H2>(d, r, R, c2, C2, V);
+}
+
+__global__ void __launch_bounds__(256) k_crop_tail_shortcut(const float* __restrict__ feat_all, int NIMG, int H, int W, int C_sc, int C_c1, int nslab,
+                                                            const float* __restrict__ rois, float stride, const float* __restrict__ bias_sc,
+                                                            float* __restrict__ sc_out) {
+  crop_roi_slab<false, 4>((int)blockIdx.x, (const float4*)feat_all, NIMG, H, W, (C_sc + C_c1) / 4, C_sc / 4, nslab, rois, stride, 7,
+                          (const float4*)bias_sc, FRCNN_ACT_NONE, (float4*)sc_out);
+}
+
+__global__ void __launch_bounds__(256) k_crop_tail_entry(const float* __restrict__ feat_all, int NIMG, int H, int W, int C_sc, int C_c1,
+                                                         const float* __restrict__ rois, int R, float stride, const float* __restrict__ bias_c1,
+                                                         const Wino7Sink<true> V) {
+  const int FC = C_sc + C_c1;
+  const int b = (int)blockIdx.x, groups = C_c1 / H2_KB;
+  const int r = __builtin_amdgcn_readfirstlane((b / groups) * 4 + ((int)threadIdx.x >> 6));
+  if (r >= R) return;
+  const int C2 = C_c1 / 2, FC2 = FC / 2;
+  const int c2 = (b % groups) * 64 + ((int)threadIdx.x & 63);
+  const float* roi = rois + 5 * (size_t)r;
+  const int img = (int)roi[0];
+  float2 d[7][7];
+  if (img < 0 || img >= NIMG) {
+#pragma unroll
+    for (int i = 0; i < 7; ++i)
+#pragma unroll
+      for (int j = 0; j < 7; ++j) d[i][j] = make_float2(0.f, 0.f);
+  } else {
+    const float height = ((float)H - 1.0f) * stride, width = ((float)W - 1.0f) * stride;
+    const float2* feat = (const float2*)feat_all + (size_t)img * H * W * FC2 + C_sc / 2;
+    const float x1 = roi[1] / width, y1 = roi[2] / height, x2 = roi[3] / width, y2 = roi[4] / height;
+    const float hs = (y2 - y1) * (float)(H - 1) / (float)(7 - 1);
+    const float ws = (x2 - x1) * (float)(W - 1) / (float)(7 - 1);
+    const float2 bv = ((const float2*)bias_c1)[c2];
+    unsigned otop[7], obot[7], oleft[7], oright[7];
+    float ly[7], lx[7];
+    bool iny[7], inx[7];
+#pragma unroll
+    for (int i = 0; i < 7; ++i) {
+      int lo, hi;
+      iny[i] = crop_axis(y1, H, hs, i, lo, hi, ly[i]);
+      otop[i] = (unsigned)lo * (unsigned)W * (unsigned)FC2;
+      obot[i] = (unsigned)hi * (unsigned)W * (unsigned)FC2;
+      inx[i] = crop_axis(x1, W, ws, i, lo, hi, lx[i]);
+      oleft[i] = (unsigned)lo * (unsigned)FC2 + (unsigned)c2;
+      oright[i] = (unsigned)hi * (unsigned)FC2 + (unsigned)c2;
+    }
+#pragma unroll
+    for (int i = 0; i < 7; ++i) {
+      float2 tl[7], tr[7], bl[7], br[7];
+#pragma unroll
+      for (int j = 0; j < 7; ++j) {
+        tl[j] = feat[otop[i] + oleft[j]]; tr[j] = feat[otop[i] + oright[j]];
+        bl[j] = feat[obot[i] + oleft[j]]; br[j] = feat[obot[i] + oright[j]];
+      }
+#pragma unroll
+      for (int j = 0; j < 7; ++j) {
+        float2 o = lerp4(lerp4(tl[j], tr[j], lx[j]), lerp4(bl[j], br[j], lx[j]), ly[i]);
+        if (!(iny[i] & inx[j])) o = make_float2(0.f, 0.f);
+        o.x += bv.x; o.y += bv.y;
+        d[i][j] = act_relu(o);
+      }
+      __builtin_amdgcn_sched_barrier(0);
+    }
+  }
+  wino7_input_body<true>(d, r, R, c2, C2, V);
 }
 
 template <int XI0, int NXI, int I0, int NI, bool H2, bool MASK>
@@ -219,6 +290,28 @@
   return FRCNN_OK;
 }
 
+extern "C" int frcnn_crop_tail_entry(const float* feat_d, int N, int H, int W, int C_sc, int C_c1, const float* rois_d, int R, float feat_stride,
+                                     int pool, const float* bias_sc_d, const float* bias_c1_d, float* sc_out_d, void* v_planes_d, float* v_inv_d,
+                                     void* stream) {
+  if (R == 0) return FRCNN_OK;
+  if (!feat_d || !rois_d || !bias_sc_d || !bias_c1_d || !sc_out_d || !v_planes_d || !v_inv_d || N <= 0 || H < 2 || W < 2 || C_sc <= 0 ||
+      C_c1 <= 0 || R < 0 || pool < 2)
+    return FRCNN_E_ARG;
+  if (pool != 7 || C_c1 % H2_KB || C_sc % 4) return FRCNN_E_UNSUPPORTED;
+  if ((long long)H * W * (C_sc + C_c1) >= (1ll << 31)) return FRCNN_E_UNSUPPORTED;
+  const int nslab = crop_roi_slabs(C_sc / 4);
+  const long long nb_sc = (long long)R * nslab, nb_c1 = (long long)((R + 3) / 4) * (C_c1 / H2_KB);
+  if (nb_sc >= (1ll << 31) || nb_c1 >= (1ll << 31) || (long long)121 * R >= (1ll << 31)) return FRCNN_E_UNSUPPORTED;
+  const Wino7Sink<true> sink{nullptr, (unsigned short*)v_planes_d, v_inv_d, (size_t)121 * R};
+  hipLaunchKernelGGL(k_crop_tail_shortcut, dim3((unsigned)nb_sc), dim3(256), 0, (hipStream_t)stream, feat_d, N, H, W, C_sc, C_c1, nslab, rois_d,
+                     feat_stride, bias_sc_d, sc_out_d);
+  LAUNCH_CHECK();
+  hipLaunchKernelGGL(k_crop_tail_entry, dim3((unsigned)nb_c1), dim3(256), 0, (hipStream_t)stream, feat_d, N, H, W, C_sc, C_c1, rois_d, R,
+                     feat_stride, bias_c1_d, sink);
+  LAUNCH_CHECK();
+  return FRCNN_OK;
+}
+
 extern "C" int frcnn_winograd7_output_transform(const float* m_d, int R, int C, const float* bias_d, int act, float* y_d, void* stream) {
   if (!m_d || !y_d || R <= 0 || C <= 0) return FRCNN_E_ARG;
   if (C % 2 || (act != FRCNN_ACT_NONE && act != FRCNN_ACT_RELU)) return FRCNN_E_UNSUPPORTED;
diff --git a/tf-faster-rcnn_amd/frcnn_hip/__init__.py b/tf-faster-rcnn_amd/frcnn_hip/__init__.py
--- a/tf-faster-rcnn_amd/frcnn_hip/__init__.py
+++ b/tf-faster-rcnn_amd/frcnn_hip/__init__.py
@@ -88,6 +88,7 @@
     "frcnn_winograd_output_transform_h2": (c_int, [_P, c_int, c_int, c_int, c_int, c_int, _P, c_int, _P, _P, _P, _P]),
     "frcnn_winograd7_input_transform_h2": (c_int, [_P, c_int, c_int, _P, _P, _P]),
     "frcnn_winograd7_output_transform_h2": (c_int, [_P, c_int, c_int, _P, c_int, _P, _P, _P, _P]),
+    "frcnn_crop_tail_entry": (c_int, [_P, c_int, c_int, c_int, c_int, c_int, _P, c_int, c_float, c_int, _P, _P, _P, _P, _P, _P]),
     "frcnn_set_tuning": (c_int, [c_int, c_int]),
     "frcnn_pack_filter_hwio": (c_int, [_P, c_int, c_int, c_int, c_int, _P, _P]),
     "frcnn_maxpool_nhwc": (c_int, [_P, c_int, c_int, c_int, c_int, c_int, c_int, c_int, c_int, _P, c_int, c_int, _P]),
diff --git a/tf-faster-rcnn_amd/frcnn_hip/ops.py b/tf-faster-rcnn_amd/frcnn_hip/ops.py
--- a/tf-faster-rcnn_amd/frcnn_hip/ops.py
+++ b/tf-faster-rcnn_amd/frcnn_hip/ops.py
@@ -337,6 +337,20 @@
     call("frcnn_crop_and_resize_bias_act", _ptr(feat), N, H, W, C, _ptr(rois), R, float(feat_stride), int(pool), _ptr(bias),
          int(act), _ptr(out), _stream())
     return out
+
+
+def crop_tail_entry(feat, rois, feat_stride, pool, c_sc, bias_sc, bias_c1, v_planes, sc_out=None):
+    _chk(feat), _chk(rois), _chk(bias_sc), _chk(bias_c1)
+    N, H, W, C = feat.shape
+    R, c_sc = rois.shape[0], int(c_sc)
+    c_c1 = C - c_sc
+    assert 0 < c_sc < C and bias_sc.numel() == c_sc and bias_c1.numel() == c_c1
+    assert isinstance(v_planes, H2) and v_planes.K == c_c1 and v_planes.rows == 121 * R
+    sc_out = _empty((R, pool, pool, c_sc), dtype=torch.float32, device=feat.device) if sc_out is None else sc_out
+    assert tuple(sc_out.shape) == (R, pool, pool, c_sc)
+    call("frcnn_crop_tail_entry", _ptr(feat), N, H, W, c_sc, c_c1, _ptr(rois), R, float(feat_stride), int(pool), _ptr(bias_sc), _ptr(bias_c1),
+         _ptr(sc_out), _ptr(v_planes.planes), _ptr(v_planes.inv), _stream())
+    return sc_out, v_planes
 
 
 def detect_post(cls_prob, bbox_pred, rois, num_rois, im_scale, im_h, im_w, nms_thresh=0.3, score_thresh=0.0,
@@ -641,17 +655,20 @@
     return out
 
 
-def conv3x3_winograd(x, u, bias, act=ACT_NONE, out=None, v_buf=None, m_buf=None, u_planes=None, v_planes=None, mask=None, out_planes=None):
-    N, H, W, Cin = x.shape
+def conv3x3_winograd(x, u, bias, act=ACT_NONE, out=None, v_buf=None, m_buf=None, u_planes=None, v_planes=None, mask=None, out_planes=None,
+                     v_ready=False):
+    N, H, W, Cin = x if v_ready else x.shape
     G, Cout = u.shape[0], u.shape[1]
     m = {16: 2, 36: 4, 121: 7}[G]
     T = winograd_tiles(N, H, W, m)
-    dev = x.device
+    assert not v_ready or (u_planes is not None and v_planes is not None)
+    dev = u.device
     mm = _empty((G, T, Cout), dtype=torch.float32, device=dev) if m_buf is None else m_buf
     out = _empty((N, H, W, Cout), dtype=torch.float32, device=dev) if out is None else out
     if u_planes is not None:
         v_planes = H2.empty(G * T, Cin, dev) if v_planes is None else v_planes
-        winograd_input_transform_h2(x, v_planes, m)
+        if not v_ready:
+            winograd_input_transform_h2(x, v_planes, m)
         gemm_h2(v_planes, u_planes, G, T, Cout, Cin, out=mm.view(G * T, Cout))
     else:
         v = _empty((G, T, Cin), dtype=torch.float32, device=dev) if v_buf is None else v_buf
diff --git a/tf-faster-rcnn_amd/frcnn_hip/runtime.py b/tf-faster-rcnn_amd/frcnn_hip/runtime.py
--- a/tf-faster-rcnn_amd/frcnn_hip/runtime.py
+++ b/tf-faster-rcnn_amd/frcnn_hip/runtime.py
@@ -402,9 +402,24 @@
             self.derived_gen += 1
         return ent[0]
 
+    def h2_planes_cat(self, name, filters):
+        key = ("h2cat", name)
+        self.prepared.wait_planes()
+        ent = self.packed.get(key)
+        if ent is None:
+            w = torch.cat([f.reshape(f.shape[0], -1) for f in filters]).contiguous()
+            ent = self.packed[key] = (w, ops.h2_pack_w(w), tuple(filters))
+            self.derived_gen += 1
+        return ent[1]
+
     def h2_refresh(self):
         for packed, w in self.h2.values():
             ops.h2_pack_w(w, packed)
+        for key, ent in self.packed.items():
+            if isinstance(key, tuple) and key and key[0] == "h2cat":
+                w, packed, filters = ent
+                torch.cat([f.reshape(f.shape[0], -1) for f in filters], out=w)
+                ops.h2_pack_w(w, packed)
 
     def h2_buf(self, name, rows, K):
         key = ("h2", name, int(rows), int(K))
diff --git a/tf-faster-rcnn_amd/lib/model/config.py b/tf-faster-rcnn_amd/lib/model/config.py
--- a/tf-faster-rcnn_amd/lib/model/config.py
+++ b/tf-faster-rcnn_amd/lib/model/config.py
@@ -56,7 +56,7 @@
              WINOGRAD_7X7=True, FUSE_TAIL_MEAN=True, MFMA_X3=True,
              MFMA_H2=True, H2_LAZY_SPLIT=True, H2_MIN_TILES=150, H2_TRAIN_MIN_TILES=320, H2_TRUNK_PLANES=True, H2_TILE_CFG=-1,
              X3_TILE_CFG=-1, H2_TRAIN=True, WGRAD_STREAM=2, WGRAD_TN=True, WGRAD_H2=True, PREP_STREAM=True, TRAIN_REPLAY=True, TRAIN_PICK_STREAMS=6,
-             GRAPH_CACHE_SHAPES=4, TRAIN_CACHE_SHAPES=16, JPEG_DEVICE=False, TEST_BATCH_IMAGES=1))
+             GRAPH_CACHE_SHAPES=4, TRAIN_CACHE_SHAPES=16, JPEG_DEVICE=False, TEST_BATCH_IMAGES=1, TAIL_ENTRY_FUSED=True))
 __C.DATA_DIR = osp.abspath(osp.join(__C.ROOT_DIR, 'data'))
 cfg = __C
 
diff --git a/tf-faster-rcnn_amd/lib/nets/network.py b/tf-faster-rcnn_amd/lib/nets/network.py
--- a/tf-faster-rcnn_amd/lib/nets/network.py
+++ b/tf-faster-rcnn_amd/lib/nets/network.py
@@ -185,10 +185,11 @@
         m = int(cfg.HIP.WINOGRAD_M)
         return 7 if (m == 4 and H == 7 and W == 7 and cfg.HIP.WINOGRAD_7X7) else m
 
-    def _conv_winograd(self, x, scope, act, bn_eps, emit_h2=False, want_f32=True):
+    def _conv_winograd(self, x, scope, act, bn_eps, emit_h2=False, want_f32=True, v_ready=False):
         sess = self._sess
-        self._need_f32(x)
-        N, H, W, Cin = x.shape
+        if not v_ready:
+            self._need_f32(x)
+        N, H, W, Cin = x if v_ready else x.shape
         m = self._winograd_scheme(scope, H, W)
         u, b = sess.winograd_params(scope, bn_eps=bn_eps, m=m)
         G, Cout = u.shape[0], u.shape[1]
@@ -196,9 +197,11 @@
         mm = sess.buf(self._tag + "/wino_m", (G, T, Cout))
         out = sess.buf(self._tag + "/" + scope, (N, H, W, Cout))
         flops = 2 * G * T * Cout * Cin
+        assert not v_ready or self._h2_eligible(T, Cout, Cin, G, scope)
         if self._h2_eligible(T, Cout, Cin, G, scope):
             vp, wp = sess.h2_buf(self._tag + "/wino_v", G * T, Cin), sess.h2_planes(u)
-            sess.mark("op:wino_in", 0, lambda: ops.winograd_input_transform_h2(x, vp, m), nbytes=4 * (x.numel() + G * T * Cin))
+            if not v_ready:
+                sess.mark("op:wino_in", 0, lambda: ops.winograd_input_transform_h2(x, vp, m), nbytes=4 * (x.numel() + G * T * Cin))
             tcfg = int(cfg.HIP.H2_TILE_CFG)
             sess.mark("conv:h2:" + scope, flops, lambda: ops.gemm_h2(vp, wp, G, T, Cout, Cin, out=mm, cfg=tcfg),
                       nbytes=4 * (G * T * Cin + mm.numel()) + 4 * u.numel())
@@ -577,7 +580,8 @@
                 c.RPN_PRE_NMS_TOP_N, c.RPN_POST_NMS_TOP_N, c.RPN_NMS_THRESH, cfg.TEST.RPN_TOP_N, cfg.POOLING_SIZE,
                 bool(cfg.HIP.WINOGRAD), int(cfg.HIP.WINOGRAD_MIN_CIN), int(cfg.HIP.WINOGRAD_M), tuple(cfg.HIP.WINOGRAD_F2_SCOPES),
                 tuple(cfg.HIP.WINOGRAD_DIRECT_SCOPES), bool(cfg.HIP.WINOGRAD_7X7), bool(cfg.HIP.FUSE_TAIL_MEAN), bool(cfg.HIP.MFMA_X3), bool(cfg.USE_E2E_TF),
-                bool(cfg.HIP.MFMA_H2), bool(cfg.HIP.H2_LAZY_SPLIT), int(cfg.HIP.H2_MIN_TILES), bool(cfg.HIP.H2_TRUNK_PLANES), int(cfg.HIP.H2_TILE_CFG), int(cfg.HIP.X3_TILE_CFG), bool(cfg.HIP.H2_TRAIN))
+                bool(cfg.HIP.MFMA_H2), bool(cfg.HIP.H2_LAZY_SPLIT), int(cfg.HIP.H2_MIN_TILES), bool(cfg.HIP.H2_TRUNK_PLANES), int(cfg.HIP.H2_TILE_CFG), int(cfg.HIP.X3_TILE_CFG), bool(cfg.HIP.H2_TRAIN),
+                bool(cfg.HIP.TAIL_ENTRY_FUSED))
 
     def shape_scope(self, sess, image_shape, im_info):
         return sess.shape_scope(self.graph_key(image_shape, im_info), group=("graphs", self._tag), cap=int(cfg.HIP.GRAPH_CACHE_SHAPES))
diff --git a/tf-faster-rcnn_amd/lib/nets/resnet_v1.py b/tf-faster-rcnn_amd/lib/nets/resnet_v1.py
--- a/tf-faster-rcnn_amd/lib/nets/resnet_v1.py
+++ b/tf-faster-rcnn_amd/lib/nets/resnet_v1.py
@@ -118,21 +118,68 @@
         c1_map = self._conv(net_conv, prefix + "/conv1", 1, 1, act=ACT_NONE, bn_eps=BN_EPS, no_bias=True)
         return sc_map, c1_map
 
+    def _tail_entry_one_launch(self, net_conv, R):
+        sess, P = self._sess, cfg.POOLING_SIZE
+        name, base, _, _ = self._blocks[-1]
+        prefix = "%s/%s/unit_1/bottleneck_v1" % (self._scope, name)
+        N, H, W, Cin = net_conv.shape
+        M, c_sc, c_c1 = N * H * W, 4 * base, base
+        if not (cfg.HIP.TAIL_ENTRY_FUSED and self._mode == "TEST" and cfg.HIP.MFMA_H2 and P == 7 and not cfg.RESNET.MAX_POOL):
+            return False
+        if c_c1 % 128 or c_sc % 4 or H * W * (c_sc + c_c1) >= (1 << 31):
+            return False
+        if not (self._h2_eligible(M, c_sc, Cin, 1, prefix + "/shortcut") and self._h2_eligible(M, c_c1, Cin, 1, prefix + "/conv1")
+                and M * (c_sc + c_c1) < (1 << 29) and 4 * (c_sc + c_c1) * Cin < (1 << 32)):
+            return False
+        scope = prefix + "/conv2"
+        wino = (cfg.HIP.WINOGRAD and c_c1 % 32 == 0 and c_c1 >= cfg.HIP.WINOGRAD_MIN_CIN
+                and not any(tok in scope for tok in cfg.HIP.WINOGRAD_DIRECT_SCOPES))
+        if not (wino and self._winograd_scheme(scope, P, P) == 7 and self._h2_eligible(R, c_c1, c_c1, 121, scope)):
+            return False
+        return self._h2_input(net_conv) is not None
+
+    def _tail_entry_planes(self, net_conv, rois):
+        sess, P = self._sess, cfg.POOLING_SIZE
+        name, base, _, _ = self._blocks[-1]
+        prefix = "%s/%s/unit_1/bottleneck_v1" % (self._scope, name)
+        N, H, W, Cin = net_conv.shape
+        M, R = N * H * W, rois.shape[0]
+        w_sc, b_sc = sess.conv_params(prefix + "/shortcut", bn_eps=BN_EPS)
+        w_c1, b_c1 = sess.conv_params(prefix + "/conv1", bn_eps=BN_EPS)
+        c_sc, c_c1 = w_sc.shape[0], w_c1.shape[0]
+        C = c_sc + c_c1
+        xp, wp = self._h2_input(net_conv), sess.h2_planes_cat(prefix + "/entry", (w_sc, w_c1))
+        emap = sess.buf(self._tag + "/" + prefix + "/entry_map", (N, H, W, C))
+        tcfg = int(cfg.HIP.H2_TILE_CFG)
+        sess.mark("conv:h2:" + prefix + "/entry", 2 * M * C * Cin,
+                  lambda: ops.gemm_h2(xp, wp, 1, M, C, Cin, None, None, ACT_NONE, out=emap, want_f32=False, cfg=tcfg),
+                  nbytes=4 * M * Cin + 4 * C * Cin + 4 * emap.numel())
+        self._wrote(emap)
+        sc_out = sess.buf(self._tag + "/" + prefix + "/shortcut_crop", (R, P, P, c_sc))
+        vp = sess.h2_buf(self._tag + "/wino_v", 121 * R, c_c1)
+        fs = float(self._feat_stride[0])
+        sess.mark("op:crop_tail_entry", 0, lambda: ops.crop_tail_entry(emap, rois, fs, P, c_sc, b_sc, b_c1, vp, sc_out),
+                  nbytes=4 * (emap.numel() + sc_out.numel() + 121 * R * c_c1))
+        return self._wrote(sc_out), (R, P, P, c_c1)
+
     def _fused_tail_entry(self, net_conv, rois):
         sess, P = self._sess, cfg.POOLING_SIZE
         name, base, n_units, stride = self._blocks[-1]
         prefix = "%s/%s/unit_1/bottleneck_v1" % (self._scope, name)
         R = rois.shape[0]
-        sc_map, c1_map = self._fused_tail_maps(net_conv)
-        b_sc = sess.conv_info[prefix + "/shortcut"]["b"]
-        b_c1 = sess.conv_info[prefix + "/conv1"]["b"]
-        fs = float(self._feat_stride[0])
-        sc_out = sess.buf(self._tag + "/" + prefix + "/shortcut_crop", (R, P, P, sc_map.shape[-1]))
-        c1_out = sess.buf(self._tag + "/" + prefix + "/conv1_crop", (R, P, P, c1_map.shape[-1]))
-        shortcut = self._crop_images(sc_map, rois, sc_out, bias=b_sc, act=ACT_NONE)
-        r = self._crop_images(c1_map, rois, c1_out, bias=b_c1, act=ACT_RELU)
         c3_h2 = self._h2_eligible(R * P * P, 4 * base, base, 1, prefix + "/conv3")
-        r = self._conv(r, prefix + "/conv2", 3, 1, (1, 1, 1, 1), act=ACT_RELU, bn_eps=BN_EPS, emit_h2=c3_h2, want_f32=not c3_h2)
+        if self._tail_entry_one_launch(net_conv, R):
+            shortcut, r_shape = self._tail_entry_planes(net_conv, rois)
+            r = self._conv_winograd(r_shape, prefix + "/conv2", ACT_RELU, BN_EPS, emit_h2=c3_h2, want_f32=not c3_h2, v_ready=True)
+        else:
+            sc_map, c1_map = self._fused_tail_maps(net_conv)
+            b_sc = sess.conv_info[prefix + "/shortcut"]["b"]
+            b_c1 = sess.conv_info[prefix + "/conv1"]["b"]
+            sc_out = sess.buf(self._tag + "/" + prefix + "/shortcut_crop", (R, P, P, sc_map.shape[-1]))
+            c1_out = sess.buf(self._tag + "/" + prefix + "/conv1_crop", (R, P, P, c1_map.shape[-1]))
+            shortcut = self._crop_images(sc_map, rois, sc_out, bias=b_sc, act=ACT_NONE)
+            r = self._crop_images(c1_map, rois, c1_out, bias=b_c1, act=ACT_RELU)
+            r = self._conv(r, prefix + "/conv2", 3, 1, (1, 1, 1, 1), act=ACT_RELU, bn_eps=BN_EPS, emit_h2=c3_h2, want_f32=not c3_h2)
         x = self._conv(r, prefix + "/conv3", 1, 1, act=ACT_RELU, bn_eps=BN_EPS, residual=shortcut, res_stride=1, emit_h2=n_units >= 2,
                        want_f32=not (n_units >= 2 and self._trunk_planes_only(R * P * P, base, stride if n_units == 2 else 1,
                                                                               "%s/%s/unit_2/bottleneck_v1" % (self._scope, name))))
```

After: 529.4 (median of 6 runs). About the same (+0.4%).
